# dhruvsreenivas/amp_extensions

Measured on AMD Instinct MI355X. Metric: learned-dynamics env steps/sec (humanoid3d, 40k-sample rollout), higher is better.
Workload: dtype fp32 (f16x3-emulated: 2 scaled fp16 limbs, 3 MFMA products per f32 MAC, fp32-level error)

## Files before the change

### amp_extensions_amd/_native.py

```python
from __future__ import annotations

import ctypes as C
import os
import re

from . import _build

_HEADER = os.path.join(_build.INCLUDE, "amx_hip.h")
ABI_VERSION = 2

c_int, c_ll, c_dbl, c_flt, c_u64, c_u32, vp = C.c_int, C.c_longlong, C.c_double, C.c_float, C.c_uint64, C.c_uint32, C.c_void_p
ip = C.POINTER(C.c_int)


class ResetNoise(C.Structure):
    _fields_ = [("noise_bef_rot", C.c_int), ("noise_min", C.c_double), ("noise_max", C.c_double),
                ("radian", C.c_double), ("rot_vel_w_pose", C.c_int), ("vel_noise", C.c_int),
                ("interp", C.c_double), ("knee_rot", C.c_int)]

    @classmethod
    def from_reset_args(cls, ra: dict) -> "ResetNoise | None":
        if float(ra["radian"]) == 0 and float(ra["noise_min"]) == 0 and float(ra["noise_max"]) == 0:
            return None
        return cls(int(bool(ra["noise_bef_rot"])), float(ra["noise_min"]), float(ra["noise_max"]),
                   float(ra["radian"]), int(bool(ra["rot_vel_w_pose"])), int(bool(ra["vel_noise"])),
                   float(ra["interp"]), int(bool(ra["knee_rot"])))


AMX_NOISE_ROT_SLOTS = 48
RFF_PART_ROWS = 32

SIGNATURES = {
    "amx_create": (vp, [c_int, c_int, c_int, c_int, c_int, c_int, c_int]),
    "amx_create_ex": (vp, [c_int, c_int, c_int, c_int, c_int, c_int, c_int, c_int]),
    "amx_destroy": (c_int, [vp]),
    "amx_last_error": (C.c_char_p, []),
    "amx_abi_version": (c_int, []),
    "amx_layout": (c_int, [vp, ip, ip, ip, ip]),
    "amx_set_normalizers": (c_int, [vp, vp, vp, vp, vp, vp, vp]),
    "amx_set_termination": (c_int, [vp, c_int, vp, vp, vp, vp, c_int, c_int, c_int, c_int, c_int,
                                    c_int, c_int, c_dbl, c_int, c_dbl]),
    "amx_assemble_input": (c_int, [vp, vp, vp, c_int, vp, c_ll, c_int, c_int, vp]),
    "amx_assemble_input_rexp": (c_int, [vp, vp, vp, c_int, vp, c_ll, c_int, c_int, vp, c_ll, c_ll, c_int, vp]),
    "amx_gemm_bias_act": (c_int, [vp, c_int, c_int, c_int, c_int, vp, c_int, c_ll, vp, c_int, c_ll,
                                  vp, c_ll, vp, c_int, c_ll, c_int, c_int, vp]),
    "amx_gemm_bias_act_t64": (c_int, [vp, c_int, c_int, c_int, c_int, vp, c_int, c_ll, vp, c_int, c_ll,
                                      vp, c_ll, vp, c_int, c_ll, c_int, c_int, vp]),
    "amx_gemm_out_unnorm": (c_int, [vp, c_int, c_int, c_int, c_int, vp, c_int, c_ll, vp, c_int, c_ll,
                                    vp, c_ll, vp, c_int, c_ll, vp]),
    "amx_split_bf16x3": (c_int, [vp, c_int, c_int, c_int, vp, c_int, c_ll, vp, c_ll, vp]),
    "amx_gemm_bias_act_x6": (c_int, [vp, c_int, c_int, c_int, c_int, vp, c_int, c_ll, vp, c_ll,
                                     vp, c_ll, vp, c_int, c_ll, c_int, c_int, vp]),
    "amx_gemm_out_unnorm_x6": (c_int, [vp, c_int, c_int, c_int, c_int, vp, c_int, c_ll, vp, c_ll,
                                       vp, c_ll, vp, c_int, c_ll, vp]),
    "amx_rff_features_x6": (c_int, [vp, c_int, c_int, c_int, c_int, vp, c_int, vp, vp, c_flt, vp, c_int,
                                    vp, vp, vp]),
    "amx_split_f16x2": (c_int, [vp, c_int, c_int, c_int, vp, c_int, c_ll, vp, c_ll, vp, c_ll, vp]),
    "amx_row_exponents": (c_int, [vp, c_int, c_int, c_int, vp, c_int, c_ll, vp, c_ll, c_int, vp]),
    "amx_gemm_bias_act_h3": (c_int, [vp, c_int, c_int, c_int, c_int, vp, c_int, c_ll, vp, c_ll, vp, c_ll,
                                     vp, c_ll, vp, c_int, c_ll, c_int, c_int, vp, c_ll, c_int, vp, c_int, vp]),
    "amx_gemm_out_unnorm_h3": (c_int, [vp, c_int, c_int, c_int, c_int, vp, c_int, c_ll, vp, c_ll, vp, c_ll,
                                       vp, c_ll, vp, c_int, c_ll, vp, c_ll, c_int, c_int, vp]),
    "amx_gemm_bias_act_h3_win": (c_int, [vp, c_int, c_int, c_int, c_int, vp, c_int, c_ll, vp, c_ll, vp, c_ll,
                                         vp, c_ll, vp, c_int, c_ll, c_int, c_int, vp, c_ll, c_int, vp, c_int, vp]),
    "amx_gemm_out_unnorm_h3_win": (c_int, [vp, c_int, c_int, c_int, c_int, vp, c_int, c_ll, vp, c_ll, vp, c_ll,
                                           vp, c_ll, vp, c_int, c_ll, vp, c_ll, c_int, vp]),
    "amx_set_motion": (c_int, [vp, vp, c_ll]),
    "amx_motion_duration": (c_dbl, [vp]),
    "amx_motion_states": (c_int, [vp, vp, c_int, c_int, vp, c_ll, vp]),
    "amx_motion_states_noise": (c_int, [vp, vp, c_int, c_int, vp, vp, c_ll, c_u64, vp, c_ll, vp]),
    "amx_reset_lanes_motion_noise": (c_int, [vp, vp, vp, c_u64, c_dbl, c_int, vp, vp, c_ll, vp, vp, vp, vp, vp, vp,
                                             c_int, vp]),
    "amx_reset_lanes_motion": (c_int, [vp, vp, vp, c_u64, c_dbl, c_int, vp, vp, vp, vp, vp, vp, c_int, vp]),
    "amx_amp_obs_size": (c_int, [vp]),
    "amx_state_amp_obs": (c_int, [vp, vp, vp, c_ll, c_int, c_int, vp, c_ll, vp]),
    "amx_motion_amp_obs": (c_int, [vp, vp, c_dbl, c_int, c_int, vp, c_ll, vp]),
    "amx_state_amp_rows": (c_int, [vp, vp, vp, c_ll, c_int, c_int, vp, c_ll, vp]),
    "amx_tw_dim": (c_int, [vp]),
    "amx_state_tw_rows": (c_int, [vp, vp, c_ll, c_int, c_int, vp, c_ll, vp]),
    "amx_motion_tw_rows": (c_int, [vp, vp, vp, c_int, c_int, c_dbl, vp, c_ll, vp]),
    "amx_dtw_work": (c_ll, [c_int, c_int]),
    "amx_dtw_align": (c_int, [vp, vp, vp, c_ll, c_int, c_int, c_int, vp, vp, c_int, c_int, vp, vp, vp, vp, vp, vp, vp]),
    "amx_npg_param_count": (c_ll, [c_int, c_int]),
    "amx_npg_pass": (c_int, [vp, c_int, c_int, vp, c_int, c_ll, vp, c_int, c_ll, vp, vp, vp, c_int, vp, vp]),
    "amx_npg_reduce": (c_int, [vp, vp, c_int, c_int, vp, vp]),
    "amx_npg_pass_gated": (c_int, [vp, c_int, c_int, vp, c_int, c_ll, vp, c_int, c_ll, vp, vp, vp, c_int, vp, vp, vp]),
    "amx_npg_reduce_gated": (c_int, [vp, vp, c_int, c_int, vp, vp, vp]),
    "amx_npg_curvature": (c_int, [vp, vp, c_int, c_int, vp, vp]),
    "amx_npg_cg_tail_work": (c_ll, [c_int]),
    "amx_npg_cg_tail": (c_int, [vp, vp, c_int, c_int, c_int, vp, c_dbl, c_dbl, vp, vp, vp, vp, vp, vp, vp, vp, vp]),
    "amx_npg_cg_reduce": (c_int, [vp, vp, c_int, c_int, c_int, vp, c_dbl, vp, vp, vp, vp, vp]),
    "amx_npg_cg_xrp": (c_int, [vp, c_int, c_dbl, vp, vp, vp, vp, vp, vp, vp, vp, vp]),
    "amx_npg_pass_cg": (c_int, [vp, c_int, vp, c_int, c_ll, vp, c_int, vp, vp, c_dbl, vp, vp, vp, vp, vp, vp, vp, vp,
                                vp, vp]),
    "amx_npg_pass_idx": (c_int, [vp, c_int, c_int, vp, vp, c_int, c_ll, vp, vp, c_int, vp, vp, vp, vp, vp]),
    "amx_npg_pass_cg_idx": (c_int, [vp, c_int, c_int, vp, vp, c_int, c_ll, vp, c_int, vp, vp, c_dbl, vp, vp, vp, vp,
                                    vp, vp, vp, vp, vp, vp, vp]),
    "amx_npg_ll_blocks": (c_int, [vp, c_int]),
    "amx_npg_ll": (c_int, [vp, c_int, vp, c_ll, vp, c_ll, vp, vp, vp, vp, vp]),
    "amx_npg_apply_step": (c_int, [vp, c_int, c_int, vp, vp, vp, c_int, c_dbl, c_dbl, c_flt, vp, vp, vp]),
    "amx_npg_pass_ex": (c_int, [vp, c_int, c_int, vp, c_int, c_ll, vp, c_int, c_ll, vp, vp, vp, c_int, vp, vp, vp, vp]),
    "amx_npg_pass_dp": (c_int, [vp, c_int, c_int, vp, c_int, c_ll, vp, c_int, c_ll, vp, vp, vp, c_int, vp, vp, vp, c_ll,
                                vp]),
    "amx_npg_pass_cg_dp": (c_int, [vp, c_int, vp, c_int, c_ll, vp, c_int, vp, vp, c_dbl, vp, vp, vp, vp, vp, vp, vp,
                                   vp, vp, c_ll, vp]),
    "amx_npg_cg_init": (c_int, [vp, c_int, vp, vp, vp, vp, vp, vp, vp]),
    "amx_npg_cg_init_ls": (c_int, [vp, c_int, c_int, vp, vp, vp, vp, vp, vp, vp, vp, vp]),
    "amx_npg_cg_step": (c_int, [vp, c_int, c_int, vp, vp, c_dbl, c_dbl, vp, vp, vp, vp, vp, vp]),
    "amx_step": (c_int, [vp, vp, c_int, c_ll, vp, vp, vp, vp, vp, vp, vp, c_int, vp, c_int, vp]),
    "amx_step_rexp": (c_int, [vp, vp, c_int, c_ll, vp, vp, vp, vp, vp, vp, vp, c_int, vp, vp, c_int, vp]),
    "amx_step_reset": (c_int, [vp, vp, c_int, c_ll, vp, vp, vp, vp, vp, vp, vp, c_int, vp, vp, vp, c_int, vp,
                               c_u64, vp, vp, vp, vp, vp, c_ll, vp, c_int, vp]),
    "amx_step_reset_act": (c_int, [vp, vp, c_int, c_ll, vp, vp, vp, vp, vp, vp, vp, c_int, vp, vp, vp, c_int, vp,
                                   c_u64, vp, vp, vp, vp, vp, vp, c_int, c_int, vp, c_u64, c_u64, vp, c_int, vp, vp,
                                   vp, c_ll, c_int, vp, c_ll, c_ll, c_int, c_int, vp]),
    "amx_set_step_act_occupancy": (c_int, [vp, c_int]),
    "amx_rff_features_h3": (c_int, [vp, c_int, c_int, c_int, c_int, vp, c_int, vp, vp, vp, vp, c_flt, vp, c_int,
                                    vp, vp, vp]),
    "amx_mlp_features_h3": (c_int, [vp, c_int, c_int, c_int, c_int, vp, c_int, vp, vp, vp, vp, c_flt, vp, c_int,
                                    vp, vp, vp]),
    "amx_disagreement": (c_int, [vp, vp, c_int, c_ll, vp, c_int, vp]),
    "amx_reset_lanes": (c_int, [vp, vp, vp, c_int, vp, c_u64, vp, vp, vp, vp, vp, vp, c_int, vp]),
    "amx_policy_act": (c_int, [vp, vp, c_int, vp, c_int, c_int, vp, vp, c_u64, c_u64, c_int, vp, vp, vp, c_ll,
                               c_int, vp, c_ll, c_ll, c_int, vp]),
    "amx_policy_act_dev": (c_int, [vp, vp, c_int, vp, c_int, c_int, vp, vp, c_u64, vp, c_u64, c_int, vp, vp, vp,
                                   c_ll, c_int, vp, c_ll, c_ll, c_int, vp]),
    "amx_counter_add": (c_int, [vp, vp, c_ll, vp]),
    "amx_set_gemm_timer": (c_int, [vp, vp]),
    "amx_split_workspace_floats": (c_ll, [vp, c_int, c_int, ip]),
    "amx_set_split_workspace": (c_int, [vp, vp, c_ll, vp, c_int]),
    "amx_policy_blob_floats": (c_ll, [vp, c_int, c_int]),
    "amx_policy_pack": (c_int, [vp, vp, vp, c_int, vp, vp, c_int, vp, vp, vp, vp]),
    "amx_rff_features": (c_int, [vp, c_int, c_int, c_int, c_int, vp, c_int, vp, c_int, vp, c_flt, vp, c_int,
                                 vp, vp, vp]),
    "amx_sum_partials": (c_int, [vp, vp, c_int, c_int, vp, vp]),
    "amx_mmd_fit": (c_int, [vp, vp, c_dbl, vp, c_int, vp, vp, vp]),
    "amx_mmd_reward": (c_int, [vp, vp, c_int, vp, c_int, vp, c_flt, c_dbl, c_flt, c_flt, vp, vp, vp, c_int, vp]),
    "amx_mmd_reward_raw": (c_int, [vp, vp, c_int, vp, c_int, vp, c_dbl, vp, vp, vp, c_int, vp]),
    "amx_expert_cost": (c_int, [vp, vp, c_int, vp, c_int, c_int, c_flt, c_flt, vp, vp, c_dbl, vp]),
    "amx_feature_message": (c_int, [vp, vp, c_int, c_int, c_dbl, vp, vp]),
    "amx_mmd_relabel": (c_int, [vp, vp, c_dbl, vp, c_int, vp, vp, vp, c_int, vp, c_flt, c_dbl, c_int, c_flt, c_flt,
                                vp, vp, vp, c_int, vp, c_int, c_int, vp, vp, vp, vp]),
    "amx_amp_reward": (c_int, [vp, vp, c_int, c_int, vp, c_flt, vp, c_dbl, vp, vp, c_int, vp]),
    "amx_disc_reward": (c_int, [vp, c_int, vp, c_int, c_int, vp, c_flt, vp, c_dbl, vp, vp, c_int, vp]),
    "amx_cost_rows": (c_int, [vp, vp, c_ll, c_int, vp, c_ll, c_int, vp, c_ll, c_int, c_int, vp, c_int, vp]),
    "amx_value_features": (c_int, [vp, c_int, c_int, vp, vp, vp, c_ll, vp, vp, c_int, vp, c_int, vp]),
    "amx_value_head": (c_int, [vp, c_int, vp, c_int, c_int, vp, vp, vp, vp]),
    "amx_gae": (c_int, [vp, c_int, c_int, vp, vp, c_ll, vp, vp, vp, c_ll, vp, c_dbl, c_dbl, vp, vp, vp]),
    "amx_adv_whiten": (c_int, [vp, c_int, c_int, vp, vp, c_ll, vp, c_dbl, vp, vp, vp]),
    "amx_adv_whiten_parts": (c_int, [vp, c_int, c_int, vp, vp, c_ll, vp, c_int, c_int, vp, vp]),
    "amx_adv_whiten_apply": (c_int, [vp, c_int, c_int, vp, vp, c_ll, vp, vp, c_int, c_dbl, vp, vp, vp]),
    "amx_vfit_work": (c_ll, [c_int, c_int, c_int]),
    "amx_vfit_param_count": (c_ll, [c_int, c_int, c_int]),
    "amx_vfit_epoch": (c_int, [vp, c_int, vp, c_int, vp, vp, c_int, c_int, c_int, vp, vp, vp, vp, vp, vp, vp, vp, vp,
                               c_dbl, c_dbl, c_dbl, c_dbl, c_dbl, vp, vp, vp]),
    "amx_efit_param_count": (c_ll, [vp]),
    "amx_efit_work_floats": (c_ll, [vp, c_int]),
    "amx_efit_step": (c_int, [vp, c_int, c_int, c_int, vp, c_ll, c_int, vp, vp, vp, vp, vp, vp, vp, vp, vp, c_int,
                              c_dbl, c_dbl, c_dbl, vp, c_ll, vp, vp]),
    "amx_gemm_nn_f32": (c_int, [vp, c_int, c_int, c_int, vp, c_int, vp, c_int, vp, c_int, vp, c_int, c_int, vp]),
    "amx_gemm_tn_f32": (c_int, [vp, c_int, c_int, c_int, vp, c_int, vp, c_int, vp, c_int, vp, c_int, vp, c_int, vp]),
    "amx_dfit_param_count": (c_ll, [c_int, c_int, c_int]),
    "amx_dfit_work_floats": (c_ll, [c_int, c_int, c_int, c_int]),
    "amx_dfit_step": (c_int, [vp, c_int, c_int, c_dbl, c_dbl, c_dbl, c_dbl, c_dbl, c_int, c_int, c_int, c_int, c_int,
                              c_int, vp, vp, vp, c_ll, c_int, vp, c_ll, c_int, vp, vp, vp, vp, vp, vp, vp, vp, vp, vp,
                              vp, vp]),
    "amx_bcfit_work": (c_ll, [c_int, c_int]),
    "amx_bcfit_steps": (c_int, [vp, c_int, vp, c_ll, vp, c_ll, vp, c_int, vp, vp, vp, vp, c_dbl, c_dbl, c_dbl, c_dbl,
                                c_dbl, c_int, vp, vp]),
    "amx_bcfit_eval": (c_int, [vp, c_int, vp, c_ll, vp, c_ll, vp, c_int, vp, vp, vp]),
    "amx_ppo_steps": (c_int, [vp, c_int, vp, c_ll, vp, c_ll, vp, vp, vp, c_int, vp, c_int, vp, vp, vp, vp, c_dbl, c_dbl,
                              c_dbl, c_dbl, c_dbl, vp, vp, vp]),
    "amx_ppo_old_ll": (c_int, [vp, c_int, vp, c_ll, vp, c_ll, vp, vp, vp]),
    "amx_philox":(c_int, [vp, c_u64, c_u32, c_u32, c_u32, vp, c_int, vp]),
    "amx_mt_seed": (c_int, [vp, c_int, vp, vp, c_int]),
    "amx_mt_policy_noise": (c_int, [vp, c_int, vp, c_int, c_int, c_int, vp, c_ll, c_ll]),
}
AMX_MT_STATE_BYTES = 2512

AMX_ROW_TILE = 128
AMX_K_TILE = 32
AMX_SHAPE_SPHERE, AMX_SHAPE_CAPSULE, AMX_SHAPE_BOX = 0, 1, 2
AMX_ACT_NONE, AMX_ACT_RELU = 0, 1
AMX_CONNECT_DENSE, AMX_CONNECT_PLAIN = 0, 1
AMX_IN_F64, AMX_IN_F32 = 0, 1
AMX_DISC_LEAST_SQUARES, AMX_DISC_LOG_LIKELIHOOD = 0, 1
AMX_EFIT_ADAM, AMX_EFIT_SGD = 0, 1
AMX_DFIT_SGD, AMX_DFIT_ADAM = 0, 1
AMX_BC_MSE, AMX_BC_MLE = 0, 1
AMX_DTW_COST_SQUARED, AMX_DTW_COST_POINTS = 0, 1
AMX_PPO_OLD_SNAPSHOT, AMX_PPO_OLD_TRACKS_MEAN = 0, 1


class AmxNativeError(RuntimeError):
    pass


def header_symbols(path: str = _HEADER) -> list[str]:
    txt = open(path).read()
    txt = re.sub(r"/\*.*?\*/", "", txt, flags=re.S)
    return sorted(set(re.findall(r"\b(amx_[a-z0-9_]+)\s*\(", txt)))


_LIB = None


def load(path: str | None = None, build_if_missing: bool = False):
    global _LIB
    if _LIB is not None and path is None:
        return _LIB
    path = path or _build.LIB_PATH
    if not os.path.exists(path):
        if build_if_missing:
            _build.build()
        else:
            raise AmxNativeError(
                f"{path} is missing: build it with `python -m amp_extensions_amd._build` "
                "(there is no CPU fallback for the rollout hot path)")
    try:
        lib = C.CDLL(path, mode=C.RTLD_GLOBAL)
    except OSError as e:
        raise AmxNativeError(f"cannot load {path}: {e}") from e
    for name, (res, args) in SIGNATURES.items():
        fn = getattr(lib, name)
        fn.restype = res
        fn.argtypes = args
    if lib.amx_abi_version() != ABI_VERSION:
        raise AmxNativeError("libamx_hip ABI version mismatch")
    if path == _build.LIB_PATH:
        _LIB = lib
    return lib


def check(rc: int, what: str = "") -> None:
    if rc != 0:
        msg = _LIB.amx_last_error().decode() if _LIB is not None else "?"
        raise AmxNativeError(f"{what or 'amx call'} failed ({rc}): {msg}")


def ptr(t) -> int | None:
    if t is None:
        return None
    return t.data_ptr()


def stream_handle(device=None) -> int:
    import torch
    return torch.cuda.current_stream(device).cuda_stream
```

### amp_extensions_amd/csrc/amx_step.hip

```cpp
#include "amx_common.h"

#include <utility>
#include <stdlib.h>

namespace {

template <int CTRL, int RM>
__device__ __forceinline__ double dpp_f64(double v) {
  const int lo = __builtin_amdgcn_update_dpp(0, __double2loint(v), CTRL, RM, 0xf, false);
  const int hi = __builtin_amdgcn_update_dpp(0, __double2hiint(v), CTRL, RM, 0xf, false);
  return __hiloint2double(hi, lo);
}

__device__ inline double wave_sum(double v) {
  v += dpp_f64<0xb1, 0xf>(v);
  v += dpp_f64<0x4e, 0xf>(v);
  v += dpp_f64<0x141, 0xf>(v);
  v += dpp_f64<0x140, 0xf>(v);
  v += dpp_f64<0x142, 0xa>(v);
  v += dpp_f64<0x143, 0xc>(v);
  const int lo = __builtin_amdgcn_readlane(__double2loint(v), 63);
  const int hi = __builtin_amdgcn_readlane(__double2hiint(v), 63);
  return __hiloint2double(hi, lo);
}

template <typename T>
__global__ __launch_bounds__(256) void k_assemble(const T* __restrict__ ob, const T* __restrict__ act,
                                                  const float* __restrict__ norm, float* __restrict__ buf,
                                                  long long stride_m, int ldk, int S, int A, int M, int k0_pad,
                                                  int B, int* __restrict__ row_exp, long long stride_rexp,
                                                  long long slot_stride, int n_slots) {
  const int b = (blockIdx.x * blockDim.x + threadIdx.x) >> 6;
  const int lane = threadIdx.x & 63;
  if (b >= B) return;
  const float* mu_s = norm;
  const float* sd_s = norm + S;
  const float* mu_a = norm + 2 * S;
  const float* sd_a = norm + 2 * S + A;
  uint32_t mx = 0;
  const int copies = stride_m == 0 ? 1 : M;
  for (int j = lane; j < k0_pad; j += 64) {
    float x = 0.f;
    if (j < S) {
      const float s = (float)ob[(long long)b * S + j];
      x = (s - mu_s[j]) / sd_s[j];
    } else if (j < S + A) {
      const int k = j - S;
      const float v = (float)act[(long long)b * A + k];
      x = (v - mu_a[k]) / sd_a[k];
    }
    for (int m = 0; m < copies; ++m) buf[m * stride_m + (long long)b * ldk + j] = x;
    const uint32_t bits = __float_as_uint(x) & 0x7fffffffu;
    mx = mx > bits ? mx : bits;
  }
  if (row_exp == nullptr) return;
#pragma unroll
  for (int off = 32; off > 0; off >>= 1) {
    const uint32_t o = (uint32_t)__shfl_xor((int)mx, off);
    mx = mx > o ? mx : o;
  }
  if (lane < n_slots) {
    int e = (int)(mx >> 23) - 126;
    e = e < -100 ? -100 : (e > 100 ? 100 : e);
    const int v = lane == 0 ? e : -100;
    if (slot_stride < B) {
      const int Bq = (int)slot_stride, g = b / Bq;
      row_exp[g * stride_rexp + lane * slot_stride + (b - g * Bq)] = v;
    } else {
      for (int m = 0; m < M; ++m) row_exp[m * stride_rexp + lane * slot_stride + b] = v;
    }
  }
}

template <int MM>
__device__ inline float lane_disagreement(const float* __restrict__ preds, long long strideP, int ldp, int b,
                                          int S, int lane) {
  constexpr int NP = MM * (MM - 1) / 2;
  double acc[NP > 0 ? NP : 1];
#pragma unroll
  for (int p = 0; p < (NP > 0 ? NP : 1); ++p) acc[p] = 0.0;
  for (int j = lane; j < S; j += 64) {
    float v[MM];
#pragma unroll
    for (int m = 0; m < MM; ++m) v[m] = preds[m * strideP + (long long)b * ldp + j];
    int p = 0;
#pragma unroll
    for (int i = 0; i < MM; ++i)
#pragma unroll
      for (int k = i + 1; k < MM; ++k) {
        const float d = v[i] - v[k];
        acc[p++] += (double)d * (double)d;
      }
  }
  double best = 0.0;
#pragma unroll
  for (int p = 0; p < NP; ++p) {
    const double n = wave_sum(acc[p]);
    best = (p == 0 || n > best) ? n : best;
  }
  return (float)sqrt(best);
}

__device__ inline float lane_disagreement_any(const float* __restrict__ preds, long long strideP, int ldp, int b,
                                              int S, int M, int lane) {
  double best = 0.0;
  bool first = true;
  for (int i = 0; i < M; ++i)
    for (int k = i + 1; k < M; ++k) {
      double acc = 0.0;
      for (int j = lane; j < S; j += 64) {
        const float d = preds[i * strideP + (long long)b * ldp + j] - preds[k * strideP + (long long)b * ldp + j];
        acc += (double)d * (double)d;
      }
      const double n = wave_sum(acc);
      best = (first || n > best) ? n : best;
      first = false;
    }
  return (float)sqrt(best);
}

__device__ inline float disagreement_dispatch(int M, const float* preds, long long strideP, int ldp, int b, int S,
                                              int lane) {
  if (M == 4) return lane_disagreement<4>(preds, strideP, ldp, b, S, lane);
  return M >= 2 ? lane_disagreement_any(preds, strideP, ldp, b, S, M, lane) : 0.f;
}

__global__ __launch_bounds__(256) void k_disagreement(const float* __restrict__ preds, long long strideP, int ldp,
                                                      float* __restrict__ disc, int S, int M, int B) {
  const int b = (blockIdx.x * blockDim.x + threadIdx.x) >> 6;
  const int lane = threadIdx.x & 63;
  if (b >= B) return;
  const float d = disagreement_dispatch(M, preds, strideP, ldp, b, S, lane);
  if (lane == 0) disc[b] = d;
}

struct StepArgs {
  const float* preds; long long strideP; int ldp;
  const int32_t* model_idx; int32_t* model_idx_out;
  const double* ob; double* ob_next;
  int32_t* num_steps; uint8_t* done; float* disc;
  float* cost_in; int ldc;
  int* cost_rexp;
  uint8_t* nonfinite;
  int S, M, B;
  amx_termination term;
  double* ob_out; const double* table; int R; const int32_t* rows; uint32_t k0, k1;
  int32_t* reset_count; int32_t* row_out;
  int32_t* steps0_out;
  uint64_t* counter; long long counter_delta;
  double* ob_rec;
};

template <int NIT, bool MM4>
__device__ __forceinline__ void step_lane(const StepArgs& a, int b, int lane, float* srow) {
  const amx_termination& T = a.term;
  const int S = a.S;
  const int k = a.model_idx[b];
  const int ns0 = a.num_steps[b];
  const int rc0 = a.ob_out ? a.reset_count[b] : 0;
  const int row0 = (a.ob_out && a.rows) ? a.rows[b] : 0;
  const double* ob = a.ob + (long long)b * S;
  double* on = a.ob_next + (long long)b * S;

  double o[NIT], x[NIT];
  float p[NIT];
  float pm[MM4 ? 4 : 1][NIT];
  if constexpr (MM4) {
    const float* pb = a.preds + (long long)b * a.ldp;
#pragma unroll
    for (int it = 0; it < NIT; ++it) {
      const int j = lane + 64 * it;
      o[it] = j < S ? ob[j] : 0.0;
#pragma unroll
      for (int m = 0; m < 4; ++m) pm[m][it] = j < S ? pb[m * a.strideP + j] : 0.f;
    }
#pragma unroll
    for (int it = 0; it < NIT; ++it)
      p[it] = k == 0 ? pm[0][it] : k == 1 ? pm[1][it] : k == 2 ? pm[2][it] : pm[3][it];
  } else {
    const float* pk = a.preds + (long long)k * a.strideP + (long long)b * a.ldp;
#pragma unroll
    for (int it = 0; it < NIT; ++it) {
      const int j = lane + 64 * it;
      o[it] = j < S ? ob[j] : 0.0;
      p[it] = j < S ? pk[j] : 0.f;
    }
  }
  const bool vscale = T.vel_check && T.record_vel_as_pos;
  bool vel_bad = false, bad = false;
  uint32_t cmax = 0;
#pragma unroll
  for (int it = 0; it < NIT; ++it) {
    const int j = lane + 64 * it;
    double v = o[it] + (double)p[it];
    if (vscale && j >= T.vel_offset) v = v / T.sampling_rate;
    x[it] = v;
    if (j < S) {
      on[j] = v;
      if (a.ob_rec) a.ob_rec[(long long)b * S + j] = o[it];
      if (T.vel_check && j >= T.vel_offset) vel_bad |= fabs(v) > T.vel_thresh;
      bad |= !isfinite(v);
      if (a.cost_in) {
        const float c0 = (float)o[it], c1 = (float)v;
        a.cost_in[(long long)b * a.ldc + j] = c0;
        a.cost_in[(long long)b * a.ldc + S + j] = c1;
        const uint32_t u0 = __float_as_uint(c0) & 0x7fffffffu, u1 = __float_as_uint(c1) & 0x7fffffffu;
        cmax = cmax > u0 ? cmax : u0;
        cmax = cmax > u1 ? cmax : u1;
      }
    }
  }
  if (a.cost_in) {
    for (int j = 2 * S + lane; j < a.ldc; j += 64) a.cost_in[(long long)b * a.ldc + j] = 0.f;
    if (a.cost_rexp) {
#pragma unroll
      for (int off = 32; off > 0; off >>= 1) {
        const uint32_t oo = (uint32_t)__shfl_xor((int)cmax, off);
        cmax = cmax > oo ? cmax : oo;
      }
      if (lane == 0) {
        int e = (int)(cmax >> 23) - 126;
        a.cost_rexp[b] = e < -100 ? -100 : (e > 100 ? 100 : e);
      }
    }
  }

  auto fetch = [&](int j) -> double {
    const int src = j & 63, itj = j >> 6;
    double r = 0.0;
#pragma unroll
    for (int it = 0; it < NIT; ++it) {
      const double v = __shfl(x[it], src);
      r = (itj == it) ? v : r;
    }
    return r;
  };
  const int bi = lane < T.n ? lane : 0;
  const double root_y = fetch(0);
  const double rel_y = fetch(T.y_index[bi]);
  const double ny = fetch(T.shape[bi] == AMX_SHAPE_CAPSULE ? T.ny_index[bi] : 0);
  bool hit = false;
  if (lane < T.n && (T.shape[bi] == AMX_SHAPE_SPHERE || T.shape[bi] == AMX_SHAPE_CAPSULE)) {
    const double y = T.list_index_world[bi] ? rel_y : root_y + rel_y;
    if (T.shape[bi] == AMX_SHAPE_SPHERE) {
      hit = y <= T.thresh[bi];
    } else {
      const double top = T.half_h[bi] * ny;
      const double bot = T.neg_half_h[bi] * ny;
      const double ytop = y + top;
      const double ybot = y + bot;
      hit = (ytop <= T.thresh[bi]) || (ybot <= T.thresh[bi]);
    }
  }
  const bool collided = __ballot(hit) != 0ull;
  const bool vexp = __ballot(vel_bad) != 0ull;
  const bool nf = __ballot(bad) != 0ull;

  float d = 0.f;
  if constexpr (MM4) {
    if (a.disc) {
      double acc[6] = {0.0, 0.0, 0.0, 0.0, 0.0, 0.0};
#pragma unroll
      for (int it = 0; it < NIT; ++it) {
        if (lane + 64 * it < S) {
          int q = 0;
#pragma unroll
          for (int i = 0; i < 4; ++i)
#pragma unroll
            for (int kk = i + 1; kk < 4; ++kk) {
              const float df = pm[i][it] - pm[kk][it];
              acc[q++] += (double)df * (double)df;
            }
        }
      }
      double mx = 0.0;
#pragma unroll
      for (int q = 0; q < 6; ++q) {
        const double n = wave_sum(acc[q]);
        mx = (q == 0 || n > mx) ? n : mx;
      }
      d = (float)sqrt(mx);
    }
  } else {
    if (a.disc) d = disagreement_dispatch(a.M, a.preds, a.strideP, a.ldp, b, S, lane);
  }

  const int ns = ns0 + 1;
  const bool horizon_done = ns >= T.horizon;
  const bool dn = horizon_done || collided || vexp;
  bool reset = false;
  if (a.ob_out) {
    double* oo = a.ob_out + (long long)b * S;
    if (!dn) {
#pragma unroll
      for (int it = 0; it < NIT; ++it) {
        const int j = lane + 64 * it;
        if (j < S) {
          oo[j] = x[it];
          if (srow) srow[j] = (float)x[it];
        }
      }
      if (lane == 0 && a.row_out) a.row_out[b] = -1;
    } else {
      reset = true;
      const int rc = rc0 + 1;
      int row;
      if (a.rows) {
        row = row0;
      } else {
        const amx::u32x4 r = amx::philox4x32_10({(uint32_t)b, (uint32_t)rc, 0u, amx::kTagReset}, a.k0, a.k1);
        row = (int)((((uint64_t)r.y << 32) | r.x) % (uint64_t)a.R);
      }
      const double* src = a.table + (long long)row * S;
      for (int j = lane; j < S; j += 64) {
        const double v = src[j];
        oo[j] = v;
        if (srow) srow[j] = (float)v;
      }
      if (lane == 0) {
        a.reset_count[b] = rc;
        a.model_idx_out[b] = rc % a.M;
        if (a.row_out) a.row_out[b] = row;
      }
    }
  }

  if (a.counter && b == 0 && lane == 0) a.counter[0] += (uint64_t)a.counter_delta;
  if (lane == 0) {
    if (a.steps0_out) a.steps0_out[b] = ns - 1;
    a.num_steps[b] = reset ? 0 : ns;
    a.done[b] = dn ? 1 : 0;
    if (a.disc) a.disc[b] = d;
    if (a.nonfinite) a.nonfinite[b] = nf ? 1 : 0;
  }
}

template <int NIT, bool MM4>
__global__ __launch_bounds__(256) void k_step(StepArgs a) {
  const int b = (blockIdx.x * blockDim.x + threadIdx.x) >> 6;
  const int lane = threadIdx.x & 63;
  if (b >= a.B) return;
  step_lane<NIT, MM4>(a, b, lane, nullptr);
}

__global__ __launch_bounds__(256) void k_reset(const uint8_t* __restrict__ mask, const double* __restrict__ table,
                                               int R, const int32_t* __restrict__ rows, uint32_t k0, uint32_t k1,
                                               const double* ob_src, double* ob_out, int32_t* num_steps,
                                               int32_t* model_idx, int32_t* reset_count, int32_t* row_out, int S,
                                               int M, int B) {
  const int b = (blockIdx.x * blockDim.x + threadIdx.x) >> 6;
  const int lane = threadIdx.x & 63;
  if (b >= B) return;
  const bool do_reset = (mask == nullptr) || mask[b] != 0;
  if (!do_reset) {
    if (ob_src != ob_out)
      for (int j = lane; j < S; j += 64) ob_out[(long long)b * S + j] = ob_src[(long long)b * S + j];
    if (lane == 0 && row_out) row_out[b] = -1;
    return;
  }
  const int rc = reset_count[b] + 1;
  int row;
  if (rows) {
    row = rows[b];
  } else {
    const amx::u32x4 r = amx::philox4x32_10({(uint32_t)b, (uint32_t)rc, 0u, amx::kTagReset}, k0, k1);
    const uint64_t x = ((uint64_t)r.y << 32) | r.x;
    row = (int)(x % (uint64_t)R);
  }
  const double* src = table + (long long)row * S;
  for (int j = lane; j < S; j += 64) ob_out[(long long)b * S + j] = src[j];
  if (lane == 0) {
    reset_count[b] = rc;
    model_idx[b] = rc % M;
    num_steps[b] = 0;
    if (row_out) row_out[b] = row;
  }
}

constexpr int POL_LANES = 16;
constexpr int POL_MAXH = 256;
constexpr int POL_X0_COLS = 320;

__host__ __device__ inline int pol_stride(int k) {
  const int r = (k + 3) & ~3;
  return (r % 8 == 0) ? r + 4 : r;
}

__host__ __device__ inline int pol_blob_floats(int S, int H1, int H2, int A) {
  const int s1 = pol_stride(S), s2 = pol_stride(H1), s3 = pol_stride(H2);
  return (H1 * s1 + H2 * s2 + A * s3 + H1 + H2 + A + 3) & ~3;
}

__host__ __device__ inline int pol_part_floats(int H1, int H2, int A) {
  int h = H1 > H2 ? H1 : H2;
  h = h > A ? h : A;
  const int w = 16 * ((h + 15) / 16);
  return POL_LANES * (w > 64 ? w : 64);
}

__host__ inline size_t pol_lds_bytes(int S, int H1, int H2, int A) {
  const int s1 = pol_stride(S), s2 = pol_stride(H1), s3 = pol_stride(H2);
  const size_t fl = (size_t)pol_blob_floats(S, H1, H2, A) + POL_LANES * (s1 + s2 + s3 + 2 * A) +
                    pol_part_floats(H1, H2, A);
  return fl * sizeof(float);
}

struct PolicyArgs {
  const double* ob; const float* blob; int H1; int H2; const double* nscale; const double* noise;
  uint32_t k0, k1, ctr_lo, ctr_hi; int eval_mode;
  const uint64_t* ctr_dev;
  double* act; float* mean_out;
  float* x0; long long stride_m; int ldk; int k0_pad; int M; const float* norm;
  int* row_exp; long long stride_rexp; long long slot_stride; int n_slots;
  int S, A, B;
};

typedef float pf4 __attribute__((ext_vector_type(4)));

constexpr int POL_STAGE_W = 12;
constexpr int POL_STAGE_O = 16;

__device__ inline void pol_zero_pads(float* __restrict__ dst, int ds, int cols, int rows) {
  const int w = ds - cols;
  for (int i = threadIdx.x; i < rows * w; i += 256) dst[(i / w) * ds + cols + i % w] = 0.f;
}

__device__ inline void pol_stage_all(float* __restrict__ img, const float* __restrict__ blob, int n4,
                                     float* __restrict__ so, int s1, const double* __restrict__ ob, int n_ob,
                                     int S) {
  const int t = threadIdx.x;
  for (int it = 0;; ++it) {
    const int w0 = t + it * 256 * POL_STAGE_W, o0 = t + it * 256 * POL_STAGE_O;
    if (w0 >= n4 && o0 >= n_ob) break;
    pf4 wv[POL_STAGE_W];
    double ov[POL_STAGE_O];
#pragma unroll
    for (int u = 0; u < POL_STAGE_W; ++u) {
      const int i = w0 + u * 256;
      if (i < n4) wv[u] = reinterpret_cast<const pf4*>(blob)[i];
    }
#pragma unroll
    for (int u = 0; u < POL_STAGE_O; ++u) {
      const int i = o0 + u * 256;
      if (i < n_ob) ov[u] = ob[i];
    }
#pragma unroll
    for (int u = 0; u < POL_STAGE_W; ++u) {
      const int i = w0 + u * 256;
      if (i < n4) reinterpret_cast<pf4*>(img)[i] = wv[u];
    }
#pragma unroll
    for (int u = 0; u < POL_STAGE_O; ++u) {
      const int i = o0 + u * 256;
      if (i < n_ob) {
        const int r = i / S, c = i - r * S;
        so[r * s1 + c] = (float)ov[u];
      }
    }
  }
}

__device__ inline int pol_ksplit(int nblk, int nc) {
  const int jjt = (nc + 3) >> 2;
  return nblk >= 4 ? 1 : (4 / nblk < jjt ? 4 / nblk : jjt);
}

__device__ inline void pol_mfma_layer(const float* __restrict__ x, int ldx, int nc, const float* __restrict__ w,
                                      int ldw, int N, float* __restrict__ part) {
  const int lane = threadIdx.x & 63, wave = threadIdx.x >> 6;
  const int i = lane & 15, kq = lane >> 4;
  const int nblk = (N + 15) >> 4, jjt = (nc + 3) >> 2, ksplit = pol_ksplit(nblk, nc);
  const int ldp = 16 * nblk;
  for (int item = wave; item < nblk * ksplit; item += 4) {
    const int nb = item % nblk, kh = item / nblk;
    const int jj0 = kh * jjt / ksplit, jj1 = (kh + 1) * jjt / ksplit;
    const int u = 16 * nb + i;
    const float* xr = x + i * ldx;
    const float* wr = w + (u < N ? u : 0) * ldw;
    pf4 acc = {0.f, 0.f, 0.f, 0.f};
    for (int jj = jj0; jj < jj1; ++jj) {
      const int c = kq + 4 * jj;
      const bool ok = c < nc;
      const pf4 a = ok ? *reinterpret_cast<const pf4*>(xr + 4 * c) : pf4{0.f, 0.f, 0.f, 0.f};
      const pf4 b = (ok && u < N) ? *reinterpret_cast<const pf4*>(wr + 4 * c) : pf4{0.f, 0.f, 0.f, 0.f};
      acc = __builtin_amdgcn_mfma_f32_16x16x4f32(a.x, b.x, acc, 0, 0, 0);
      acc = __builtin_amdgcn_mfma_f32_16x16x4f32(a.y, b.y, acc, 0, 0, 0);
      acc = __builtin_amdgcn_mfma_f32_16x16x4f32(a.z, b.z, acc, 0, 0, 0);
      acc = __builtin_amdgcn_mfma_f32_16x16x4f32(a.w, b.w, acc, 0, 0, 0);
    }
    float* pp = part + kh * 16 * ldp + 16 * nb + i;
#pragma unroll
    for (int r = 0; r < 4; ++r) pp[(4 * kq + r) * ldp] = acc[r];
  }
}

__device__ inline void pol_combine(const float* __restrict__ part, int N, int nc, const float* __restrict__ bias,
                                   bool tanh_act, float* __restrict__ out, int ldo) {
  const int nblk = (N + 15) >> 4, ksplit = pol_ksplit(nblk, nc), ldp = 16 * nblk;
  for (int e = threadIdx.x; e < POL_LANES * N; e += 256) {
    const int l = e / N, u = e - l * N;
    float z = part[l * ldp + u];
    for (int kh = 1; kh < ksplit; ++kh) z += part[(kh * 16 + l) * ldp + u];
    z = z + bias[u];
    out[l * ldo + u] = tanh_act ? tanhf(z) : z;
  }
}

__device__ __forceinline__ void policy_core(const PolicyArgs& p, float* psm, int b0, int img_floats) {
  const int S = p.S, A = p.A, H1 = p.H1, H2 = p.H2;
  const int s1 = pol_stride(S), s2 = pol_stride(H1), s3 = pol_stride(H2);
  float* w1 = psm;
  float* w2 = w1 + H1 * s1;
  float* w3 = w2 + H2 * s2;
  float* bb1 = w3 + A * s3;
  float* bb2 = bb1 + H1;
  float* bb3 = bb2 + H2;
  float* so = psm + img_floats;
  float* h1 = so + POL_LANES * s1;
  float* h2 = h1 + POL_LANES * s2;
  float* mo = h2 + POL_LANES * s3;
  float* xa_s = mo + POL_LANES * A;
  float* part = xa_s + POL_LANES * A;
  const int t = threadIdx.x;
  const bool on = t < 256;
  const int nc1 = (S + 3) >> 2, nc2 = (H1 + 3) >> 2, nc3 = (H2 + 3) >> 2;
  const int npairs = (A + 1) >> 1;
  constexpr int POL_PRE = 2;
  double pre_n[POL_PRE][2], pre_s[POL_PRE][2];
#pragma unroll
  for (int q = 0; q < POL_PRE; ++q) {
    const int e = t + 256 * q;
    const int l = e / npairs, pr = e - l * npairs, b = b0 + l;
#pragma unroll
    for (int h = 0; h < 2; ++h) {
      const int u = 2 * pr + h;
      const bool ok = on && e < POL_LANES * npairs && b < p.B && u < A;
      pre_n[q][h] = (ok && p.noise && !p.eval_mode) ? p.noise[(long long)b * A + u] : 0.0;
      pre_s[q][h] = (ok && !p.eval_mode) ? p.nscale[u] : 0.0;
    }
  }
  if (on) pol_mfma_layer(so, s1, nc1, w1, s1, H1, part);
  __syncthreads();
  if (on) pol_combine(part, H1, nc1, bb1, true, h1, s2);
  __syncthreads();
  if (on) pol_mfma_layer(h1, s2, nc2, w2, s2, H2, part);
  __syncthreads();
  if (on) pol_combine(part, H2, nc2, bb2, true, h2, s3);
  __syncthreads();
  if (on) pol_mfma_layer(h2, s3, nc3, w3, s3, A, part);
  __syncthreads();
  if (on) pol_combine(part, A, nc3, bb3, false, mo, A);
  __syncthreads();
  uint32_t ctr_lo = p.ctr_lo, ctr_hi = p.ctr_hi;
  if (p.ctr_dev) {
    const uint64_t cv = *p.ctr_dev + ((uint64_t)p.ctr_hi << 32 | p.ctr_lo);
    ctr_lo = (uint32_t)cv;
    ctr_hi = (uint32_t)(cv >> 32);
  }
  auto act_item = [&](int e, const double* pn, const double* ps) {
    const int l = e / npairs, pr = e - l * npairs;
    const int b = b0 + l;
    if (b >= p.B) return;
    double n[2] = {0.0, 0.0};
    if (!p.eval_mode && !p.noise) {
      const amx::u32x4 r = amx::philox4x32_10(
          {(uint32_t)b, ctr_lo, ((uint32_t)pr << 8) | (ctr_hi & 0xffu), amx::kTagPolicy}, p.k0, p.k1);
      const double u1 = 1.0 - amx::u53(r.x, r.y);
      const double u2 = amx::u53(r.z, r.w);
      const double rad = sqrt(-2.0 * log(u1));
      const double ang = 6.283185307179586 * u2;
      n[0] = rad * cos(ang);
      n[1] = rad * sin(ang);
    }
#pragma unroll
    for (int h = 0; h < 2; ++h) {
      const int u = 2 * pr + h;
      if (u >= A) break;
      const float m = mo[l * A + u];
      if (p.mean_out) p.mean_out[(long long)b * A + u] = m;
      double a_out;
      if (p.eval_mode) {
        a_out = (double)m;
      } else {
        const double nz = p.noise ? (pn ? pn[h] : p.noise[(long long)b * A + u]) : n[h];
        a_out = (double)m + (ps ? ps[h] : p.nscale[u]) * nz;
      }
      p.act[(long long)b * A + u] = a_out;
      if (p.x0) xa_s[l * A + u] = (float)a_out;
    }
  };
  if (on) {
#pragma unroll
    for (int q = 0; q < POL_PRE; ++q)
      if (t + 256 * q < POL_LANES * npairs) act_item(t + 256 * q, pre_n[q], pre_s[q]);
    for (int e = t + 256 * POL_PRE; e < POL_LANES * npairs; e += 256) act_item(e, nullptr, nullptr);
  }
  if (!p.x0) return;
  __syncthreads();
  if (!on) return;
  const float* mu_s = p.norm;
  const float* sd_s = p.norm + S;
  const float* mu_a = p.norm + 2 * S;
  const float* sd_a = p.norm + 2 * S + A;
  const int k0 = p.k0_pad;
  const int copies = p.stride_m == 0 ? 1 : p.M;
  const int ll = t >> 4, c0 = t & 15;
  const int bb = b0 + ll;
  const bool row_ok = bb < p.B;
  constexpr int QT = POL_X0_COLS / 16;
  float mu[QT], sd[QT];
#pragma unroll
  for (int q = 0; q < QT; ++q) {
    const int j = c0 + 16 * q;
    mu[q] = 0.f;
    sd[q] = 1.f;
    if (j < S) {
      mu[q] = mu_s[j];
      sd[q] = sd_s[j];
    } else if (j < S + A) {
      mu[q] = mu_a[j - S];
      sd[q] = sd_a[j - S];
    }
  }
  uint32_t mx = 0;
  if (row_ok) {
#pragma unroll
    for (int q = 0; q < QT; ++q) {
      const int j = c0 + 16 * q;
      if (j >= k0) break;
      float x = 0.f;
      if (j < S) {
        x = (so[ll * s1 + j] - mu[q]) / sd[q];
      } else if (j < S + A) {
        x = (xa_s[ll * A + j - S] - mu[q]) / sd[q];
      }
      for (int mm = 0; mm < copies; ++mm) p.x0[mm * p.stride_m + (long long)bb * p.ldk + j] = x;
      const uint32_t bits = __float_as_uint(x) & 0x7fffffffu;
      mx = mx > bits ? mx : bits;
    }
  }
  if (p.row_exp == nullptr) return;
#pragma unroll
  for (int off = 8; off > 0; off >>= 1) {
    const uint32_t o = (uint32_t)__shfl_xor((int)mx, off);
    mx = mx > o ? mx : o;
  }
  if (!row_ok) return;
  int e = (int)(mx >> 23) - 126;
  e = e < -100 ? -100 : (e > 100 ? 100 : e);
  for (int sl = c0; sl < p.n_slots; sl += 16) {
    const int v = sl == 0 ? e : -100;
    if (p.slot_stride < p.B) {
      const int Bq = (int)p.slot_stride, g = bb / Bq;
      p.row_exp[g * p.stride_rexp + sl * p.slot_stride + (bb - g * Bq)] = v;
    } else {
      for (int mm = 0; mm < p.M; ++mm) p.row_exp[mm * p.stride_rexp + sl * p.slot_stride + bb] = v;
    }
  }
}


__global__ __launch_bounds__(256) void k_policy(PolicyArgs p) {
  extern __shared__ __attribute__((aligned(16))) float psm[];
  const int S = p.S, s1 = pol_stride(S), s2 = pol_stride(p.H1), s3 = pol_stride(p.H2);
  const int nblob = pol_blob_floats(S, p.H1, p.H2, p.A);
  float* so = psm + nblob;
  float* h1 = so + POL_LANES * s1;
  const int t = threadIdx.x;
  const int b0 = blockIdx.x * POL_LANES;
  const int nl = (p.B - b0) < POL_LANES ? (p.B - b0) : POL_LANES;
  pol_zero_pads(so, s1, S, nl);
  for (int i = t + nl * s1; i < POL_LANES * s1; i += 256) so[i] = 0.f;
  pol_stage_all(psm, p.blob, nblob >> 2, so, s1, p.ob + (long long)b0 * S, nl * S, S);
  for (int i = t; i < POL_LANES * (s2 + s3); i += 256) h1[i] = 0.f;
  __syncthreads();
  policy_core(p, psm, b0, nblob);
}

__host__ __device__ inline int pol_image_lds_floats(int S, int H1, int H2, int A) {
  return (pol_blob_floats(S, H1, H2, A) + 255) & ~255;
}

template <int NIT, bool MM4, bool W8>
__global__ __launch_bounds__(1024) __attribute__((amdgpu_waves_per_eu(W8 ? 8 : 1))) void k_step_act(StepArgs a,
                                                                                                    PolicyArgs p) {
  extern __shared__ __attribute__((aligned(16))) float psm[];
  const int S = p.S, s1 = pol_stride(S), s2 = pol_stride(p.H1), s3 = pol_stride(p.H2);
  const int nimg = pol_image_lds_floats(S, p.H1, p.H2, p.A);
  float* so = psm + nimg;
  float* h1 = so + POL_LANES * s1;
  const int t = threadIdx.x, lane = t & 63, wave = t >> 6;
  const int b0 = blockIdx.x * POL_LANES, b = b0 + wave;
  for (int q = wave; q < (nimg >> 8); q += POL_LANES)
    __builtin_amdgcn_global_load_lds((const __attribute__((address_space(1))) void*)(p.blob + q * 256 + 4 * lane),
                                     (__attribute__((address_space(3))) void*)(psm + q * 256), 16, 0, 0);
  float* srow = so + wave * s1;
  if (b < a.B) {
    step_lane<NIT, MM4>(a, b, lane, srow);
    for (int j = S + lane; j < s1; j += 64) srow[j] = 0.f;
  } else {
    for (int j = lane; j < s1; j += 64) srow[j] = 0.f;
  }
  for (int i = t; i < POL_LANES * (s2 + s3); i += 1024) h1[i] = 0.f;
  __syncthreads();
  policy_core(p, psm, b0, nimg);
}

__global__ void k_policy_pack(const float* __restrict__ W1, const float* __restrict__ b1, int H1,
                              const float* __restrict__ W2, const float* __restrict__ b2, int H2,
                              const float* __restrict__ W3, const float* __restrict__ b3, int S, int A,
                              float* __restrict__ blob) {
  const int s1 = pol_stride(S), s2 = pol_stride(H1), s3 = pol_stride(H2);
  const int n = pol_blob_floats(S, H1, H2, A);
  const int i = blockIdx.x * blockDim.x + threadIdx.x;
  if (i >= n) return;
  int j = i;
  float v = 0.f;
  if (j < H1 * s1) {
    const int r = j / s1, c = j % s1;
    v = c < S ? W1[(long long)r * S + c] : 0.f;
  } else if ((j -= H1 * s1) < H2 * s2) {
    const int r = j / s2, c = j % s2;
    v = c < H1 ? W2[r * H1 + c] : 0.f;
  } else if ((j -= H2 * s2) < A * s3) {
    const int r = j / s3, c = j % s3;
    v = c < H2 ? W3[r * H2 + c] : 0.f;
  } else if ((j -= A * s3) < H1) {
    v = b1[j];
  } else if ((j -= H1) < H2) {
    v = b2[j];
  } else if ((j -= H2) < A) {
    v = b3[j];
  }
  blob[i] = v;
}

__global__ void k_philox(uint32_t k0, uint32_t k1, uint32_t c1, uint32_t c2, uint32_t c3, uint32_t* out, int n) {
  const int i = blockIdx.x * blockDim.x + threadIdx.x;
  if (i >= n) return;
  const amx::u32x4 r = amx::philox4x32_10({(uint32_t)i, c1, c2, c3}, k0, k1);
  out[4 * i + 0] = r.x;
  out[4 * i + 1] = r.y;
  out[4 * i + 2] = r.z;
  out[4 * i + 3] = r.w;
}

inline dim3 lanes_grid(int B) { return dim3((unsigned)((B + 3) / 4)); }

}

static bool blocked_rexp_ok(const amx_ctx* ctx, int B, long long stride_m, long long stride_rexp, long long slot_stride,
                            int n_slots) {
  return ctx && stride_m == 0 && slot_stride > 0 && B % slot_stride == 0 && B / slot_stride <= ctx->M &&
         stride_rexp >= (long long)n_slots * slot_stride;
}

static int assemble(const char* fn, amx_ctx* ctx, const void* ob, const void* act, int in_dtype, float* act_buf,
                    long long stride_m, int ldk, int B, int* row_exp, long long stride_rexp, long long slot_stride,
                    int n_slots, void* stream) {
  AMX_CHECK_ARG(ctx && ctx->have_norm, "%s: context has no normalizers", fn);
  AMX_CHECK_ARG(ob && act && act_buf, "%s: null pointer", fn);
  AMX_CHECK_ARG(B >= 0, "%s: B=%d", fn, B);
  AMX_CHECK_ARG(ldk >= ctx->k0_pad, "%s: ldk=%d < k0_pad=%d", fn, ldk, ctx->k0_pad);
  AMX_CHECK_ARG(ctx->M == 1 || stride_m == 0 || stride_m >= (long long)ldk * B, "%s: stride_m too small", fn);
  if (B == 0) return AMX_OK;
  hipStream_t s = (hipStream_t)stream;
  if (in_dtype == AMX_IN_F64) {
    hipLaunchKernelGGL(k_assemble<double>, lanes_grid(B), dim3(256), 0, s, (const double*)ob, (const double*)act,
                       ctx->d_norm, act_buf, stride_m, ldk, ctx->S, ctx->A, ctx->M, ctx->k0_pad, B, row_exp,
                       stride_rexp, slot_stride, n_slots);
  } else if (in_dtype == AMX_IN_F32) {
    hipLaunchKernelGGL(k_assemble<float>, lanes_grid(B), dim3(256), 0, s, (const float*)ob, (const float*)act,
                       ctx->d_norm, act_buf, stride_m, ldk, ctx->S, ctx->A, ctx->M, ctx->k0_pad, B, row_exp,
                       stride_rexp, slot_stride, n_slots);
  } else {
    AMX_CHECK_ARG(false, "%s: in_dtype=%d", fn, in_dtype);
  }
  AMX_CHECK_LAUNCH();
  return AMX_OK;
}

extern "C" int amx_assemble_input(amx_ctx* ctx, const void* ob, const void* act, int in_dtype, float* act_buf,
                                  long long stride_m, int ldk, int B, void* stream) {
  return assemble("amx_assemble_input", ctx, ob, act, in_dtype, act_buf, stride_m, ldk, B, nullptr, 0, 0, 0,
                  stream);
}

extern "C" int amx_assemble_input_rexp(amx_ctx* ctx, const void* ob, const void* act, int in_dtype, float* act_buf,
                                       long long stride_m, int ldk, int B, int* row_exp, long long strideRexp,
                                       long long slot_stride, int n_slots, void* stream) {
  AMX_CHECK_ARG(row_exp && n_slots >= 1 && n_slots <= 64 &&
                    (slot_stride >= B ? (ctx == nullptr || ctx->M == 1 || strideRexp >= (long long)n_slots * slot_stride)
                                      : blocked_rexp_ok(ctx, B, stride_m, strideRexp, slot_stride, n_slots)),
                "amx_assemble_input_rexp: row_exp=%p n_slots=%d slot_stride=%lld strideRexp=%lld B=%d", (void*)row_exp,
                n_slots, slot_stride, strideRexp, B);
  return assemble("amx_assemble_input_rexp", ctx, ob, act, in_dtype, act_buf, stride_m, ldk, B, row_exp, strideRexp,
                  slot_stride, n_slots, stream);
}

static int make_policy_args(const char* fn, amx_ctx* ctx, const double* ob, int B, const float* blob, int H1, int H2,
                            const double* noise_scale, const double* noise, uint64_t seed, uint64_t counter,
                            const uint64_t* counter_dev, int eval_mode, double* act, float* mean, float* x0_buf,
                            long long stride_m, int ldk, int* row_exp, long long stride_rexp, long long slot_stride,
                            int n_slots, PolicyArgs& p) {
  AMX_CHECK_ARG(ctx && blob && act, "%s: null pointer", fn);
  AMX_CHECK_ARG(amx::aligned16(blob), "%s: blob must be 16-byte aligned", fn);
  AMX_CHECK_ARG(eval_mode || noise_scale, "%s: noise_scale required unless eval_mode", fn);
  AMX_CHECK_ARG(H1 > 0 && H1 <= POL_MAXH && H2 > 0 && H2 <= POL_MAXH && ctx->A <= POL_MAXH && ctx->S <= POL_MAXH,
                "%s: S=%d H1=%d H2=%d A=%d (max %d)", fn, ctx->S, H1, H2, ctx->A, POL_MAXH);
  AMX_CHECK_ARG(B >= 0, "%s: B=%d", fn, B);
  AMX_CHECK_ARG(!x0_buf || ctx->k0_pad <= POL_X0_COLS, "%s: fused assembly needs k0_pad <= %d (%d)", fn,
                POL_X0_COLS, ctx->k0_pad);
  AMX_CHECK_ARG(!x0_buf || (ctx->have_norm && ldk >= ctx->k0_pad &&
                            (ctx->M == 1 || stride_m == 0 || stride_m >= (long long)ldk * B)),
                "%s: fused assembly needs normalizers and ldk >= k0_pad, stride_m >= ldk*B", fn);
  AMX_CHECK_ARG(!row_exp || (x0_buf && n_slots >= 1 && n_slots <= 64 &&
                             (slot_stride >= B ? (ctx->M == 1 || stride_rexp >= (long long)n_slots * slot_stride)
                                               : blocked_rexp_ok(ctx, B, stride_m, stride_rexp, slot_stride, n_slots))),
                "%s: row_exp needs x0_buf, 1 <= n_slots <= 64, slot_stride >= B (or the member-blocked layout), "
                "stride_rexp", fn);
  const size_t lds = pol_lds_bytes(ctx->S, H1, H2, ctx->A);
  AMX_CHECK_ARG(lds <= 160 * 1024, "%s: S/H too large for LDS staging (%zu B)", fn, lds);
  p.ob = ob; p.blob = blob; p.H1 = H1; p.H2 = H2;
  p.nscale = noise_scale; p.noise = noise;
  p.k0 = (uint32_t)seed; p.k1 = (uint32_t)(seed >> 32); p.ctr_lo = (uint32_t)counter;
  p.ctr_hi = (uint32_t)(counter >> 32); p.eval_mode = eval_mode; p.ctr_dev = counter_dev;
  p.act = act; p.mean_out = mean;
  p.x0 = x0_buf; p.stride_m = stride_m; p.ldk = ldk; p.k0_pad = ctx->k0_pad; p.M = ctx->M; p.norm = ctx->d_norm;
  p.row_exp = row_exp; p.stride_rexp = stride_rexp; p.slot_stride = slot_stride; p.n_slots = n_slots;
  p.S = ctx->S; p.A = ctx->A; p.B = B;
  return AMX_OK;
}

static int policy_act(amx_ctx* ctx, const double* ob, int B, const float* blob, int H1, int H2,
                      const double* noise_scale, const double* noise, uint64_t seed, uint64_t counter,
                      const uint64_t* counter_dev, int eval_mode, double* act, float* mean, float* x0_buf,
                      long long stride_m, int ldk, int* row_exp, long long stride_rexp, long long slot_stride,
                      int n_slots, void* stream) {
  AMX_CHECK_ARG(ob, "amx_policy_act: null ob");
  PolicyArgs p;
  const int rc = make_policy_args("amx_policy_act", ctx, ob, B, blob, H1, H2, noise_scale, noise, seed, counter,
                                  counter_dev, eval_mode, act, mean, x0_buf, stride_m, ldk, row_exp, stride_rexp,
                                  slot_stride, n_slots, p);
  if (rc) return rc;
  if (B == 0) return AMX_OK;
  hipLaunchKernelGGL(k_policy, dim3((B + POL_LANES - 1) / POL_LANES), dim3(256), pol_lds_bytes(ctx->S, H1, H2, ctx->A),
                     (hipStream_t)stream, p);
  AMX_CHECK_LAUNCH();
  return AMX_OK;
}

struct ResetArgs {
  const double* table; int R; const int32_t* rows; uint64_t seed; double* ob_out; int32_t* model_idx;
  int32_t* reset_count; int32_t* row_out; int32_t* steps0_out;
  uint64_t* counter; long long counter_delta; double* ob_rec;
};

static int step_impl(amx_ctx* ctx, const float* preds, int ldp, long long strideP, const int32_t* model_idx,
                     const double* ob, double* ob_next, int32_t* num_steps, uint8_t* done, float* disc,
                     float* cost_in, int ldc, int* cost_rexp, uint8_t* nonfinite, int B, void* stream,
                     const ResetArgs* rs = nullptr, const PolicyArgs* pa = nullptr) {
  AMX_CHECK_ARG(ctx && ctx->have_term, "amx_step: context has no termination config");
  AMX_CHECK_ARG(preds && model_idx && ob && ob_next && num_steps && done, "amx_step: null pointer");
  AMX_CHECK_ARG(ldp >= ctx->S && B >= 0, "amx_step: ldp=%d B=%d", ldp, B);
  AMX_CHECK_ARG(!disc || ctx->M >= 2, "amx_step: disagreement needs >= 2 models");
  AMX_CHECK_ARG(!cost_in || ldc >= 2 * ctx->S, "amx_step: ldc=%d < 2S", ldc);
  AMX_CHECK_ARG(ob != ob_next, "amx_step: ob and ob_next must not alias");
  if (B == 0) return AMX_OK;
  StepArgs a;
  a.preds = preds; a.strideP = strideP; a.ldp = ldp;
  a.model_idx = model_idx; a.ob = ob; a.ob_next = ob_next;
  a.num_steps = num_steps; a.done = done; a.disc = disc;
  a.cost_in = cost_in; a.ldc = ldc; a.cost_rexp = cost_rexp; a.nonfinite = nonfinite;
  a.S = ctx->S; a.M = ctx->M; a.B = B; a.term = ctx->term;
  a.model_idx_out = nullptr; a.ob_out = nullptr; a.table = nullptr; a.R = 0; a.rows = nullptr; a.k0 = a.k1 = 0;
  a.reset_count = nullptr; a.row_out = nullptr; a.steps0_out = nullptr; a.counter = nullptr; a.counter_delta = 0;
  a.ob_rec = nullptr;
  if (rs) {
    AMX_CHECK_ARG(rs->table && rs->ob_out && rs->model_idx && rs->reset_count && rs->R > 0,
                  "amx_step_reset: null reset pointer or R=%d", rs->R);
    AMX_CHECK_ARG(rs->ob_out != ob_next && (const int32_t*)rs->model_idx == model_idx,
                  "amx_step_reset: ob_out must differ from ob_next and model_idx be the step's");
    AMX_CHECK_ARG(rs->ob_rec == nullptr || (rs->ob_rec != ob && rs->ob_rec != ob_next && rs->ob_rec != rs->ob_out),
                  "amx_step_reset: ob_rec must be a fourth buffer");
    a.model_idx_out = rs->model_idx; a.ob_out = rs->ob_out; a.table = rs->table; a.R = rs->R; a.rows = rs->rows;
    a.k0 = (uint32_t)rs->seed; a.k1 = (uint32_t)(rs->seed >> 32);
    a.reset_count = rs->reset_count; a.row_out = rs->row_out; a.steps0_out = rs->steps0_out;
    a.counter = rs->counter; a.counter_delta = rs->counter_delta; a.ob_rec = rs->ob_rec;
  }
  const int nit = (ctx->S + 63) / 64;
  if (pa) {
    AMX_CHECK_ARG(rs && !rs->counter && !pa->noise && pa->B == B && nit <= 4,
                  "amx_step_reset_act: needs the table reset, no counter advance, no injected noise, S <= 256");
    const size_t lds = pol_lds_bytes(ctx->S, pa->H1, pa->H2, ctx->A) +
                       (size_t)(pol_image_lds_floats(ctx->S, pa->H1, pa->H2, ctx->A) -
                                pol_blob_floats(ctx->S, pa->H1, pa->H2, ctx->A)) * sizeof(float);
    AMX_CHECK_ARG(lds <= 160 * 1024, "amx_step_reset_act: S/H too large for LDS staging (%zu B)", lds);
    const dim3 grid((B + POL_LANES - 1) / POL_LANES);
    switch (nit) {
#define AMX_STEP_ACT_CASE(N)                                                                                       \
  case N:                                                                                                          \
    if (ctx->M == 4 && ctx->step_act_w8) hipLaunchKernelGGL((k_step_act<N, true, true>), grid, dim3(1024), lds,     \
                                                           (hipStream_t)stream, a, *pa);                          \
    else if (ctx->M == 4) hipLaunchKernelGGL((k_step_act<N, true, false>), grid, dim3(1024), lds, (hipStream_t)stream, \
                                             a, *pa);                                                              \
    else hipLaunchKernelGGL((k_step_act<N, false, false>), grid, dim3(1024), lds, (hipStream_t)stream, a, *pa);   \
    break;
      AMX_STEP_ACT_CASE(1) AMX_STEP_ACT_CASE(2) AMX_STEP_ACT_CASE(3) AMX_STEP_ACT_CASE(4)
#undef AMX_STEP_ACT_CASE
    }
    AMX_CHECK_LAUNCH();
    return AMX_OK;
  }
  switch (nit) {
#define AMX_STEP_CASE(N)                                                                                 \
  case N:                                                                                                \
    if (ctx->M == 4) hipLaunchKernelGGL((k_step<N, true>), lanes_grid(B), dim3(256), 0, (hipStream_t)stream, a); \
    else hipLaunchKernelGGL((k_step<N, false>), lanes_grid(B), dim3(256), 0, (hipStream_t)stream, a);     \
    break;
    AMX_STEP_CASE(1) AMX_STEP_CASE(2) AMX_STEP_CASE(3) AMX_STEP_CASE(4)
    AMX_STEP_CASE(5) AMX_STEP_CASE(6) AMX_STEP_CASE(7) AMX_STEP_CASE(8)
#undef AMX_STEP_CASE
    default: AMX_CHECK_ARG(false, "amx_step: S=%d exceeds 512", ctx->S);
  }
  AMX_CHECK_LAUNCH();
  return AMX_OK;
}

extern "C" int amx_step(amx_ctx* ctx, const float* preds, int ldp, long long strideP, const int32_t* model_idx,
                        const double* ob, double* ob_next, int32_t* num_steps, uint8_t* done, float* disc,
                        float* cost_in, int ldc, uint8_t* nonfinite, int B, void* stream) {
  return step_impl(ctx, preds, ldp, strideP, model_idx, ob, ob_next, num_steps, done, disc, cost_in, ldc, nullptr,
                   nonfinite, B, stream);
}

extern "C" int amx_step_rexp(amx_ctx* ctx, const float* preds, int ldp, long long strideP, const int32_t* model_idx,
                             const double* ob, double* ob_next, int32_t* num_steps, uint8_t* done, float* disc,
                             float* cost_in, int ldc, int* cost_rexp, uint8_t* nonfinite, int B, void* stream) {
  AMX_CHECK_ARG(cost_in && cost_rexp, "amx_step_rexp: cost_in and cost_rexp are required");
  return step_impl(ctx, preds, ldp, strideP, model_idx, ob, ob_next, num_steps, done, disc, cost_in, ldc, cost_rexp,
                   nonfinite, B, stream);
}

extern "C" int amx_step_reset(amx_ctx* ctx, const float* preds, int ldp, long long strideP, int32_t* model_idx,
                              const double* ob, double* ob_next, int32_t* num_steps, uint8_t* done, float* disc,
                              float* cost_in, int ldc, int* cost_rexp, uint8_t* nonfinite, const double* table,
                              int R, const int32_t* rows, uint64_t seed, double* ob_out, int32_t* reset_count,
                              int32_t* row_out, int32_t* steps0_out, uint64_t* counter, long long counter_delta,
                              double* ob_rec, int B, void* stream) {
  AMX_CHECK_ARG(!cost_rexp || cost_in, "amx_step_reset: cost_rexp needs cost_in");
  const ResetArgs rs = {table, R, rows, seed, ob_out, model_idx, reset_count, row_out, steps0_out, counter,
                        counter_delta, ob_rec};
  return step_impl(ctx, preds, ldp, strideP, model_idx, ob, ob_next, num_steps, done, disc, cost_in, ldc, cost_rexp,
                   nonfinite, B, stream, &rs);
}

extern "C" int amx_step_reset_act(amx_ctx* ctx, const float* preds, int ldp, long long strideP, int32_t* model_idx,
                                  const double* ob, double* ob_next, int32_t* num_steps, uint8_t* done, float* disc,
                                  float* cost_in, int ldc, int* cost_rexp, uint8_t* nonfinite, const double* table,
                                  int R, const int32_t* rows, uint64_t seed, double* ob_out, int32_t* reset_count,
                                  int32_t* row_out, int32_t* steps0_out, double* ob_rec, const float* blob, int H1,
                                  int H2, const double* noise_scale, uint64_t policy_seed, uint64_t counter,
                                  const uint64_t* counter_dev, int eval_mode, double* act, float* mean,
                                  float* x0_buf, long long stride_m, int ldk, int* row_exp, long long stride_rexp,
                                  long long slot_stride, int n_slots, int B, void* stream) {
  AMX_CHECK_ARG(!cost_rexp || cost_in, "amx_step_reset_act: cost_rexp needs cost_in");
  PolicyArgs p;
  int rc = make_policy_args("amx_step_reset_act", ctx, nullptr, B, blob, H1, H2, noise_scale, nullptr, policy_seed,
                            counter, counter_dev, eval_mode, act, mean, x0_buf, stride_m, ldk, row_exp, stride_rexp,
                            slot_stride, n_slots, p);
  if (rc) return rc;
  const ResetArgs rs = {table, R, rows, seed, ob_out, model_idx, reset_count, row_out, steps0_out, nullptr, 0,
                        ob_rec};
  return step_impl(ctx, preds, ldp, strideP, model_idx, ob, ob_next, num_steps, done, disc, cost_in, ldc, cost_rexp,
                   nonfinite, B, stream, &rs, &p);
}

extern "C" int amx_disagreement(amx_ctx* ctx, const float* preds, int ldp, long long strideP, float* disc, int B,
                                void* stream) {
  AMX_CHECK_ARG(ctx && preds && disc, "amx_disagreement: null pointer");
  AMX_CHECK_ARG(ctx->M >= 2, "amx_disagreement: needs >= 2 models (M=%d)", ctx->M);
  AMX_CHECK_ARG(ldp >= ctx->S && B >= 0, "amx_disagreement: ldp=%d B=%d", ldp, B);
  if (B == 0) return AMX_OK;
  hipLaunchKernelGGL(k_disagreement, lanes_grid(B), dim3(256), 0, (hipStream_t)stream, preds, strideP, ldp, disc,
                     ctx->S, ctx->M, B);
  AMX_CHECK_LAUNCH();
  return AMX_OK;
}

extern "C" int amx_reset_lanes(amx_ctx* ctx, const uint8_t* mask, const double* table, int R, const int32_t* rows,
                               uint64_t seed, const double* ob_src, double* ob_out, int32_t* num_steps,
                               int32_t* model_idx, int32_t* reset_count, int32_t* row_out, int B, void* stream) {
  AMX_CHECK_ARG(ctx && table && ob_out && num_steps && model_idx && reset_count, "amx_reset_lanes: null pointer");
  AMX_CHECK_ARG(R > 0 && B >= 0, "amx_reset_lanes: R=%d B=%d", R, B);
  AMX_CHECK_ARG(mask == nullptr || ob_src != nullptr, "amx_reset_lanes: masked reset needs ob_src");
  if (B == 0) return AMX_OK;
  hipLaunchKernelGGL(k_reset, lanes_grid(B), dim3(256), 0, (hipStream_t)stream, mask, table, R, rows,
                     (uint32_t)seed, (uint32_t)(seed >> 32), ob_src, ob_out, num_steps, model_idx, reset_count,
                     row_out, ctx->S, ctx->M, B);
  AMX_CHECK_LAUNCH();
  return AMX_OK;
}

extern "C" long long amx_policy_blob_floats(const amx_ctx* ctx, int H1, int H2) {
  if (!ctx || H1 <= 0 || H2 <= 0) return -1;
  return pol_image_lds_floats(ctx->S, H1, H2, ctx->A);
}

extern "C" int amx_policy_pack(amx_ctx* ctx, const float* W1, const float* b1, int H1, const float* W2,
                               const float* b2, int H2, const float* W3, const float* b3, float* blob,
                               void* stream) {
  AMX_CHECK_ARG(ctx && W1 && b1 && W2 && b2 && W3 && b3 && blob, "amx_policy_pack: null pointer");
  AMX_CHECK_ARG(H1 > 0 && H1 <= POL_MAXH && H2 > 0 && H2 <= POL_MAXH && ctx->A <= POL_MAXH,
                "amx_policy_pack: H1=%d H2=%d A=%d (max %d)", H1, H2, ctx->A, POL_MAXH);
  AMX_CHECK_ARG(amx::aligned16(blob), "amx_policy_pack: blob must be 16-byte aligned");
  const int n = pol_blob_floats(ctx->S, H1, H2, ctx->A);
  hipLaunchKernelGGL(k_policy_pack, dim3((n + 255) / 256), dim3(256), 0, (hipStream_t)stream, W1, b1, H1, W2, b2,
                     H2, W3, b3, ctx->S, ctx->A, blob);
  AMX_CHECK_LAUNCH();
  return AMX_OK;
}

extern "C" int amx_policy_act(amx_ctx* ctx, const double* ob, int B, const float* blob, int H1, int H2,
                              const double* noise_scale, const double* noise, uint64_t seed, uint64_t counter,
                              int eval_mode, double* act, float* mean, float* x0_buf, long long stride_m, int ldk,
                              int* row_exp, long long stride_rexp, long long slot_stride, int n_slots,
                              void* stream) {
  return policy_act(ctx, ob, B, blob, H1, H2, noise_scale, noise, seed, counter, nullptr, eval_mode, act, mean,
                    x0_buf, stride_m, ldk, row_exp, stride_rexp, slot_stride, n_slots, stream);
}

extern "C" int amx_policy_act_dev(amx_ctx* ctx, const double* ob, int B, const float* blob, int H1, int H2,
                                  const double* noise_scale, const double* noise, uint64_t seed,
                                  const uint64_t* counter, uint64_t counter_offset, int eval_mode, double* act,
                                  float* mean, float* x0_buf, long long stride_m, int ldk, int* row_exp,
                                  long long stride_rexp, long long slot_stride, int n_slots, void* stream) {
  AMX_CHECK_ARG(counter, "amx_policy_act_dev: null counter");
  return policy_act(ctx, ob, B, blob, H1, H2, noise_scale, noise, seed, counter_offset, counter, eval_mode, act,
                    mean, x0_buf, stride_m, ldk, row_exp, stride_rexp, slot_stride, n_slots, stream);
}

__global__ void k_counter_add(uint64_t* c, long long d) { c[0] += (uint64_t)d; }

extern "C" int amx_counter_add(amx_ctx* ctx, uint64_t* counter, long long delta, void* stream) {
  AMX_CHECK_ARG(ctx && counter, "amx_counter_add: null pointer");
  hipLaunchKernelGGL(k_counter_add, dim3(1), dim3(1), 0, (hipStream_t)stream, counter, delta);
  AMX_CHECK_LAUNCH();
  return AMX_OK;
}

extern "C" int amx_philox(amx_ctx* ctx, uint64_t seed, uint32_t ctr1, uint32_t ctr2, uint32_t ctr3, uint32_t* out,
                          int n, void* stream) {
  AMX_CHECK_ARG(ctx && out && n >= 0, "amx_philox: bad argument");
  if (n == 0) return AMX_OK;
  hipLaunchKernelGGL(k_philox, dim3((n + 255) / 256), dim3(256), 0, (hipStream_t)stream, (uint32_t)seed,
                     (uint32_t)(seed >> 32), ctr1, ctr2, ctr3, out, n);
  AMX_CHECK_LAUNCH();
  return AMX_OK;
}

extern "C" int amx_set_step_act_occupancy(amx_ctx* ctx, int two_per_cu) {
  AMX_CHECK_ARG(ctx, "amx_set_step_act_occupancy: null ctx");
  ctx->step_act_w8 = two_per_cu ? 1 : 0;
  return AMX_OK;
}
```

### amp_extensions_amd/rollout.py

```python
from __future__ import annotations

import ctypes as C
import math

import numpy as np
import torch

from . import _native as N
from .costs import GAILCost, RBFLinearCost, input_width
from .engine import DeviceEnsemble, round_up
from .humanoid import TerminationConfig
from .policy import DevicePolicy


_CAPTURE_MODE = "thread_local"

class RolloutEngine:
    def __init__(self, ensemble: DeviceEnsemble, reset_table, lanes: int, term: TerminationConfig | None = None,
                 policy: DevicePolicy | None = None, cost=None, seed: int = 0, max_steps: int = 16,
                 eval_mode: bool = False, auto_reset: bool = True, record_means: bool = False):
        self.ens = ensemble
        self.ctx = c = ensemble.ctx
        self.term = term or TerminationConfig()
        c.set_termination(self.term)
        self.B = int(lanes)
        self.Bp = round_up(self.B, 128)
        self.K = int(max_steps)
        self.policy = policy
        self.cost = cost
        self.eval_mode = eval_mode
        self.auto_reset = auto_reset
        self.fuse_reset = True
        self.fuse_assembly = False
        self.fuse_step_act = False
        self._act_ready = -1
        self.seed = int(seed) & 0xFFFFFFFFFFFFFFFF
        dev = c.device
        from .motion import ReferenceMotion
        self.motion = reset_table if isinstance(reset_table, ReferenceMotion) else None
        self.reset_time_max = 0.0
        self.table = None
        if self.motion is None:
            table = torch.as_tensor(reset_table, dtype=torch.float64)
            if table.dim() != 2 or table.shape[1] != c.S:
                raise ValueError(f"reset table must be [R, {c.S}] float64 (or a ReferenceMotion)")
            self.table = table.to(dev).contiguous()
        S, A, B, Bp, K = c.S, c.A, self.B, self.Bp, self.K
        z = lambda *shape, dt=torch.float32: torch.zeros(*shape, dtype=dt, device=dev)
        self.obs = z(K + 1, B, S, dt=torch.float64)
        self.next_obs = z(K, B, S, dt=torch.float64) if auto_reset else self.obs[1:]
        self.acts = z(K, B, A, dt=torch.float64)
        self.done = z(K, B, dt=torch.uint8)
        self.disc = z(K, Bp)
        self.rewards = z(K, Bp)
        self.ipm = z(K, Bp)
        self.wbonus = z(K, Bp)
        self.nonfinite = z(K, B, dt=torch.uint8)
        self.num_steps = z(B, dt=torch.int32)
        self.steps0 = z(B, dt=torch.int32)
        self.model_idx = z(B, dt=torch.int32)
        self.reset_count = z(B, dt=torch.int32)
        self.reset_rows = z(K, B, dt=torch.int32)
        self.reset_times = z(K, B, dt=torch.float64) if self.motion is not None else None
        self.cost_type = getattr(cost, "input_type", "ss") if cost is not None else "ss"
        if isinstance(cost, RBFLinearCost):
            self.kc = cost.map.Kp
        elif isinstance(cost, GAILCost):
            self.kc = cost.Kin
        else:
            self.kc = c.k_rff_pad
        if cost is not None:
            width = input_width(self.cost_type, S, A, getattr(cost, "motion", None))
            if cost.input_dim != width:
                raise ValueError(f"cost input width {cost.input_dim} does not match input_type "
                                 f"{self.cost_type!r} (S={S}, A={A}: {width})")
        self.cost_in = z(K, Bp, self.kc)
        if self.cost_type == "amp" and cost.motion.ctx is not c:
            raise ValueError("the cost's ReferenceMotion must live on the engine's context")
        self.row_mask = None
        if B != Bp:
            self.row_mask = ((torch.arange(K * Bp, device=dev) % Bp) < B).to(torch.uint8)
        self._scored = 0
        self.means = z(K, B, A) if record_means else None
        self.cost_rexp = None
        if (isinstance(cost, RBFLinearCost) and cost.map.W2 is not None) or \
                (isinstance(cost, GAILCost) and cost.gemm == "f16x3"):
            self.cost_rexp = z(K, Bp, dt=torch.int32)
        if isinstance(cost, RBFLinearCost):
            self.phi = z(K, Bp, cost.feature_dim)
            self.partials = z(K, Bp // N.RFF_PART_ROWS, cost.feature_dim, dt=torch.float64)
        self.t = 0
        self.step_counter = 0
        self.dev_step = torch.zeros(1, dtype=torch.int64, device=dev)
        self._capturing = False
        self._ctr_delta = 0
        self._ctr_folded = False
        self._carry = 0
        self._pending = None
        self._graph_ahead = False
        self._fbuf = z(cost.feature_dim + 1, dt=torch.float64) if isinstance(cost, RBFLinearCost) else None
        if self._fbuf is not None:
            self.phi_sum = self._fbuf[:cost.feature_dim]
        self.mb_mmd = None
        self.score_overlap = False
        self._side = None
        self.member_blocks = 0

    def reset_all(self, rows: torch.Tensor | None = None) -> None:
        self.reset_lanes(None, rows)

    def set_reset_noise(self, reset_args: dict | None) -> None:
        noise = N.ResetNoise.from_reset_args(reset_args) if reset_args is not None else None
        if noise is not None and self.motion is None:
            raise NotImplementedError("reset noise needs a ReferenceMotion reset source (AddNoise perturbs the "
                                      "kinematic pose / velocity, which a reset-state table does not hold)")
        self._reset_noise = noise

    def _reset_motion(self, mask, times, src, dst, t_out) -> None:
        c = self.ctx
        noise = getattr(self, "_reset_noise", None)
        N.check(c.lib.amx_reset_lanes_motion_noise(c.h, None if mask is None else mask.data_ptr(),
                                                   None if times is None else times.data_ptr(), self.seed,
                                                   float(self.reset_time_max), self.motion.kernel_flags,
                                                   None if noise is None else C.byref(noise), None, 0,
                                                   src.data_ptr(), dst.data_ptr(),
                                                   self.num_steps.data_ptr(), self.model_idx.data_ptr(),
                                                   self.reset_count.data_ptr(),
                                                   None if t_out is None else t_out.data_ptr(),
                                                   self.B, c.stream), "amx_reset_lanes_motion_noise")

    def reset_lanes(self, mask: torch.Tensor | None, rows: torch.Tensor | None = None,
                    t_out: torch.Tensor | None = None) -> None:
        c = self.ctx
        self.begin_rollout()
        dst = self.obs[0]
        if self.motion is not None:
            self._reset_motion(mask, rows, dst, dst, t_out)
            self.t = 0
            return
        N.check(c.lib.amx_reset_lanes(c.h, None if mask is None else mask.data_ptr(), self.table.data_ptr(),
                                      self.table.shape[0], None if rows is None else rows.data_ptr(), self.seed,
                                      dst.data_ptr(), dst.data_ptr(), self.num_steps.data_ptr(),
                                      self.model_idx.data_ptr(), self.reset_count.data_ptr(), None, self.B,
                                      c.stream), "amx_reset_lanes")
        self.t = 0

    def _rollout_begin(self) -> None:
        fused = self.auto_reset and self.motion is None and self.fuse_reset
        if fused and self.t != 0:
            self._carry, self.t, self._scored = self.t, 0, 0
        else:
            self.begin_rollout()

    def begin_rollout(self) -> None:
        if self.t != 0:
            self.obs[0].copy_(self.obs[self.t])
        self.t = 0
        self._scored = 0

    def sync_step_counter(self, to_device: bool = False) -> None:
        if self._graph_ahead:
            self.step_counter = int(self.dev_step.item())
            self._graph_ahead = False
        if to_device:
            self.dev_step.fill_(self.step_counter)

    def step(self, actions: torch.Tensor | None = None, reset_rows: torch.Tensor | None = None,
             noise: torch.Tensor | None = None, act_next: bool = False) -> int:
        front = self._step_front(actions, noise)
        if front[0] == 0 and self._pending is not None:
            pending, self._pending = self._pending, None
            pending()
        fuse = act_next and actions is None and noise is None and reset_rows is None and self._can_act_next()
        return self._step_back(front, reset_rows, act_next=fuse)

    def _can_act_next(self) -> bool:
        return (self.fuse_step_act and self.policy is not None and self.auto_reset and self.motion is None
                and self.fuse_reset and self.ens.W2 is not None and self.ens.shared_x0
                and self.ctx.S <= 256
                and self.t + 1 < self.K)

    def _step_front(self, actions, noise):
        c, t, B = self.ctx, self.t, self.B
        if t >= self.K:
            raise RuntimeError(f"rollout buffer full ({self.K} steps): call begin_rollout()")
        s = c.stream
        fused = self.auto_reset and self.motion is None and self.fuse_reset
        if t == 0 and not fused:
            self.steps0.copy_(self.num_steps)
        src = self._carry if (t == 0 and self._carry) else t
        self._carry = 0
        ob, ob_next, act = self.obs[src], self.next_obs[t], self.acts[t]
        x0_ready = False
        if self._act_ready == t and actions is None and noise is None:
            x0_ready = True
            self._act_ready = -1
        elif actions is not None:
            self._act_ready = -1
            act.copy_(actions)
        else:
            self._act_ready = -1
            if self.policy is None:
                raise RuntimeError("no policy and no actions given")
            if self._graph_ahead and not self._capturing:
                self.sync_step_counter()
            fuse_x0 = self.fuse_assembly and self.ens.W2 is not None and self.ens.shared_x0
            if not fuse_x0:
                ws = None
            elif self.member_blocks:
                ws = self.ens.workspace_blocked(self.member_blocks)
            else:
                ws = self.ens.workspace(B)
            self.policy.act(ob, B, act, t if self._capturing else self.step_counter, noise=noise,
                            eval_mode=self.eval_mode, mean_out=None if self.means is None else self.means[t],
                            counter_dev=self.dev_step if self._capturing else None,
                            x0=None if ws is None else ws["act"], row_exp=None if ws is None else ws["rexp"],
                            shared_x0=fuse_x0)
            x0_ready = fuse_x0
        if self.member_blocks:
            if self.B != self.ctx.M * self.member_blocks:
                raise ValueError("member-blocked stepping needs M * member_blocks lanes")
            return t, src, self.ens.forward_blocked(ob, act, self.member_blocks, x0_ready=x0_ready)
        preds = self.ens.forward_preds(ob, act, B, x0_ready=x0_ready)
        return t, src, preds

    def _step_back(self, front, reset_rows, act_next: bool = False) -> int:
        c, B, s = self.ctx, self.B, self.ctx.stream
        t, src, preds = front
        fused = self.auto_reset and self.motion is None and self.fuse_reset
        ob, ob_next = self.obs[src], self.next_obs[t]
        sP = 0 if self.member_blocks else preds.shape[1] * c.S
        disc = self.disc[t].data_ptr() if c.M >= 2 and not self.member_blocks else None
        if fused and act_next:
            ss = self.cost_type == "ss"
            pol, ws = self.policy, self.ens.workspace(B)
            rx = ws["rexp"]
            N.check(c.lib.amx_step_reset_act(
                c.h, preds.data_ptr(), c.S, sP, self.model_idx.data_ptr(), ob.data_ptr(),
                ob_next.data_ptr(), self.num_steps.data_ptr(), self.done[t].data_ptr(),
                disc, self.cost_in[t].data_ptr() if ss else None, self.kc,
                self.cost_rexp[t].data_ptr() if ss and self.cost_rexp is not None else None,
                self.nonfinite[t].data_ptr(), self.table.data_ptr(), self.table.shape[0], None, self.seed,
                self.obs[t + 1].data_ptr(), self.reset_count.data_ptr(), self.reset_rows[t].data_ptr(),
                self.steps0.data_ptr() if t == 0 else None, self.obs[0].data_ptr() if src != t else None,
                pol.blob.data_ptr(), pol.H1, pol.H2, pol.noise_scale.data_ptr(), pol.seed,
                (t + 1) if self._capturing else (self.step_counter + 1) & 0xFFFFFFFFFFFFFFFF,
                self.dev_step.data_ptr() if self._capturing else None, int(self.eval_mode), self.acts[t + 1].data_ptr(),
                None if self.means is None else self.means[t + 1].data_ptr(), ws["act"].data_ptr(), 0, c.ldk,
                rx.data_ptr(), rx.stride(0), rx.stride(1), rx.shape[1], B, s), "amx_step_reset_act")
            self._ctr_folded = False
            self._act_ready = t + 1
        elif fused:
            ss = self.cost_type == "ss"
            last = self._capturing and self._ctr_delta and t == self._ctr_delta - 1
            ctr, ctr_delta = (self.dev_step, self._ctr_delta) if last else (None, 0)
            N.check(c.lib.amx_step_reset(c.h, preds.data_ptr(), c.S, sP, self.model_idx.data_ptr(),
                                         ob.data_ptr(), ob_next.data_ptr(), self.num_steps.data_ptr(),
                                         self.done[t].data_ptr(), disc,
                                         self.cost_in[t].data_ptr() if ss else None, self.kc,
                                         self.cost_rexp[t].data_ptr() if ss and self.cost_rexp is not None else None,
                                         self.nonfinite[t].data_ptr(), self.table.data_ptr(), self.table.shape[0],
                                         None if reset_rows is None else reset_rows.data_ptr(), self.seed,
                                         self.obs[t + 1].data_ptr(), self.reset_count.data_ptr(),
                                         self.reset_rows[t].data_ptr(), self.steps0.data_ptr() if t == 0 else None,
                                         ctr.data_ptr() if ctr is not None else None, ctr_delta,
                                         self.obs[0].data_ptr() if src != t else None, B, s),
                    "amx_step_reset")
            self._ctr_folded = ctr is not None
        elif self.cost_type == "ss" and self.cost_rexp is not None:
            N.check(c.lib.amx_step_rexp(c.h, preds.data_ptr(), c.S, sP, self.model_idx.data_ptr(),
                                        ob.data_ptr(), ob_next.data_ptr(), self.num_steps.data_ptr(),
                                        self.done[t].data_ptr(), disc,
                                        self.cost_in[t].data_ptr(), self.kc, self.cost_rexp[t].data_ptr(),
                                        self.nonfinite[t].data_ptr(), B, s), "amx_step_rexp")
        else:
            N.check(c.lib.amx_step(c.h, preds.data_ptr(), c.S, sP, self.model_idx.data_ptr(),
                                   ob.data_ptr(), ob_next.data_ptr(), self.num_steps.data_ptr(),
                                   self.done[t].data_ptr(), disc,
                                   self.cost_in[t].data_ptr() if self.cost_type == "ss" else None, self.kc,
                                   self.nonfinite[t].data_ptr(), B, s), "amx_step")
        if self.cost is not None and self.cost_type != "ss":
            self._record_cost_input(t)
        if fused:
            pass
        elif self.auto_reset and self.motion is not None:
            self._reset_motion(self.done[t], reset_rows, ob_next, self.obs[t + 1], self.reset_times[t])
        elif self.auto_reset:
            N.check(c.lib.amx_reset_lanes(c.h, self.done[t].data_ptr(), self.table.data_ptr(), self.table.shape[0],
                                          None if reset_rows is None else reset_rows.data_ptr(), self.seed,
                                          ob_next.data_ptr(), self.obs[t + 1].data_ptr(), self.num_steps.data_ptr(),
                                          self.model_idx.data_ptr(), self.reset_count.data_ptr(),
                                          self.reset_rows[t].data_ptr(), B, s), "amx_reset_lanes")
        elif ob_next.data_ptr() != self.obs[t + 1].data_ptr():
            self.obs[t + 1].copy_(ob_next)
        self.t += 1
        self.step_counter += 1
        return t

    def _record_cost_input(self, t: int) -> None:
        c, B, S, A = self.ctx, self.B, self.ctx.S, self.ctx.A
        ob, nx, act = self.obs[t], self.next_obs[t], self.acts[t]
        typ = self.cost_type
        if typ == "amp":
            N.check(c.lib.amx_state_amp_rows(c.h, ob.data_ptr(), nx.data_ptr(), S, B, 0,
                                             self.cost_in[t].data_ptr(), self.kc, c.stream), "amx_state_amp_rows")
            return
        if typ == "sa":
            segs = ((ob, S, S), (act, A, A), (None, 0, 0))
        elif typ == "sas":
            segs = ((ob, S, S), (act, A, A), (nx, S, S))
        else:
            segs = ((ob, S, S), (None, 0, 0), (None, 0, 0))
        args = []
        for x, ld, w in segs:
            args += [None if x is None else x.data_ptr(), ld, w]
        N.check(c.lib.amx_cost_rows(c.h, *args, B, self.cost_in[t].data_ptr(), self.kc, c.stream), "amx_cost_rows")

    def rollout(self, K: int | None = None) -> int:
        K = self.K if K is None else K
        self._rollout_begin()
        self._act_ready = -1
        side = self._score_stream() if (self.score_overlap and K > 1 and isinstance(self.cost, RBFLinearCost)
                                        and self.cost.map.step_invariant) else None
        for t in range(K):
            self.step(act_next=t + 1 < K)
            if side is not None and t + 1 < K:
                side.wait_stream(torch.cuda.current_stream(self.ctx.device))
                with torch.cuda.stream(side):
                    self.score()
        if side is not None:
            torch.cuda.current_stream(self.ctx.device).wait_stream(side)
        self.score()
        return K * self.B

    def _score_stream(self):
        if self._side is None:
            self._side = torch.cuda.Stream(self.ctx.device)
        return self._side

    def score(self) -> None:
        c, cost, t0, t1, Bp = self.ctx, self.cost, self._scored, self.t, self.Bp
        if t1 <= t0 or cost is None:
            self._scored = t1
            return
        rows = (t1 - t0) * Bp
        x = self.cost_in[t0:t1].view(rows, self.kc)
        if isinstance(cost, RBFLinearCost):
            mask = None if self.row_mask is None else self.row_mask[t0 * Bp:t1 * Bp]
            rexp = None
            if self.cost_rexp is not None and self.cost_type == "ss":
                rexp = self.cost_rexp[t0:t1].view(rows)
            cost.map.features(x, rows, rows, self.phi[t0:t1].view(rows, -1),
                              self.partials[t0:t1].view(rows // N.RFF_PART_ROWS, -1), row_mask=mask, row_exp=rexp)
        elif isinstance(cost, GAILCost):
            rexp = None
            if self.cost_rexp is not None and self.cost_type == "ss":
                rexp = self.cost_rexp[t0:t1].view(rows)
            cost.rewards_from_input(x, rows, rows, self.disc[t0:t1].view(rows) if c.M >= 2 else None,
                                    out=self.rewards[t0:t1].view(rows), row_exp=rexp)
        self._scored = t1

    def feature_sum(self) -> torch.Tensor:
        self.relabel_pre()
        return self.phi_sum

    def relabel(self, allreduce=None) -> dict:
        cost = self.cost
        self.flush_relabel()
        self.score()
        if isinstance(cost, GAILCost):
            return {}
        if not isinstance(cost, RBFLinearCost):
            raise RuntimeError("relabel needs an RBFLinearCost or GAILCost")
        self.relabel_pre()
        if allreduce is not None:
            allreduce(self._fbuf)
        return self.relabel_post()

    def relabel_pre(self) -> torch.Tensor:
        self.score()
        c, cost = self.ctx, self.cost
        n_parts = self.t * (self.Bp // N.RFF_PART_ROWS)
        N.check(c.lib.amx_feature_message(c.h, self.partials.data_ptr(), n_parts, cost.feature_dim,
                                          float(self.t * self.B), self._fbuf.data_ptr(), c.stream),
                "amx_feature_message")
        return self._fbuf

    def relabel_post(self, T: int | None = None) -> dict:
        cost = self.cost
        n = (self.t if T is None else T) * self.Bp
        self.mb_mmd = cost.relabel_device(self._fbuf, self.phi.data_ptr(), cost.feature_dim, self.disc.data_ptr(),
                                          float(self.ens.threshold), self.rewards.data_ptr(), self.ipm.data_ptr(),
                                          self.wbonus.data_ptr(), n)
        return {"mb_mmd": self.mb_mmd}

    def graph_rollout(self, T: int | None = None, allreduce=None, tail=None, before_relabel=None, after=None):
        T = self.K if T is None else T
        if self.t != T:
            raise RuntimeError("run one eager rollout(T) before capturing")
        mmd = isinstance(self.cost, RBFLinearCost)
        c = self.ctx
        self.sync_step_counter(to_device=True)
        graphs = [torch.cuda.CUDAGraph(), torch.cuda.CUDAGraph()]
        side = torch.cuda.Stream(c.device)
        side.wait_stream(torch.cuda.current_stream(c.device))
        with torch.cuda.stream(side):
            self._capturing = True
            self._ctr_delta, self._ctr_folded = T, False
            try:
                with torch.cuda.graph(graphs[0], stream=side, capture_error_mode=_CAPTURE_MODE):
                    self.rollout(T)
                    if not self._ctr_folded:
                        N.check(c.lib.amx_counter_add(c.h, self.dev_step.data_ptr(), T, c.stream), "amx_counter_add")
                    if mmd:
                        self.relabel_pre()
                        if allreduce is None:
                            self.relabel_post()
                    if tail is not None and (allreduce is None or not mmd):
                        tail()
                if mmd and allreduce is not None:
                    with torch.cuda.graph(graphs[1], stream=side, capture_error_mode=_CAPTURE_MODE):
                        self.relabel_post()
                        if tail is not None:
                            tail()
            finally:
                self._capturing = False
                self._ctr_delta = 0
        torch.cuda.current_stream(c.device).wait_stream(side)
        self._graph_ahead = True
        two = mmd and allreduce is not None

        def replay():
            graphs[0].replay()
            if two:
                if before_relabel is not None:
                    before_relabel()
                allreduce(self._fbuf)
                graphs[1].replay()
            if after is not None:
                after()
            self._graph_ahead = True
            return T * self.B
        return replay

    def rollout_overlapped(self, T: int, allreduce_async, tail=None) -> int:
        if not isinstance(self.cost, RBFLinearCost):
            raise RuntimeError("rollout_overlapped is the MMD path (RBFLinearCost)")
        self.rollout(T)
        self.relabel_pre()
        h = allreduce_async(self._fbuf)

        def pending():
            h.wait()
            self.relabel_post(T)
            if tail is not None:
                tail()
        self._pending = pending
        return T * self.B

    def flush_relabel(self) -> None:
        if self._pending is not None:
            pending, self._pending = self._pending, None
            pending()

    def graph_rollout_overlapped(self, T: int, allreduce_async, tail=None, before_relabel=None, after=None):
        if not isinstance(self.cost, RBFLinearCost):
            raise RuntimeError("graph_rollout_overlapped is the MMD path (RBFLinearCost)")
        if self.t != T or self._pending is not None:
            raise RuntimeError("run one eager rollout(T) + relabel before capturing")
        fused = self.auto_reset and self.motion is None and self.fuse_reset
        if not fused:
            raise RuntimeError("graph_rollout_overlapped needs the fused step + table reset")
        c = self.ctx
        self.sync_step_counter(to_device=True)
        graphs = [torch.cuda.CUDAGraph() for _ in range(3)]
        side = torch.cuda.Stream(c.device)
        side.wait_stream(torch.cuda.current_stream(c.device))
        with torch.cuda.stream(side):
            self._capturing = True
            self._ctr_delta, self._ctr_folded = T, False
            try:
                with torch.cuda.graph(graphs[0], stream=side, capture_error_mode=_CAPTURE_MODE):
                    self._rollout_begin()
                    front = self._step_front(None, None)
                with torch.cuda.graph(graphs[1], stream=side, capture_error_mode=_CAPTURE_MODE):
                    self.relabel_post(T)
                    if tail is not None:
                        tail()
                    self._step_back(front, None)
                    for _ in range(T - 1):
                        self.step()
                    self.score()
                    if not self._ctr_folded:
                        N.check(c.lib.amx_counter_add(c.h, self.dev_step.data_ptr(), T, c.stream), "amx_counter_add")
                    self.relabel_pre()
                with torch.cuda.graph(graphs[2], stream=side, capture_error_mode=_CAPTURE_MODE):
                    self.relabel_post(T)
                    if tail is not None:
                        tail()
            finally:
                self._capturing = False
                self._ctr_delta = 0
        torch.cuda.current_stream(c.device).wait_stream(side)
        self._graph_ahead = True
        state = {"h": None}

        def replay():
            graphs[0].replay()
            if state["h"] is not None:
                state["h"].wait()
            if before_relabel is not None:
                before_relabel()
            graphs[1].replay()
            state["h"] = allreduce_async(self._fbuf)
            if after is not None:
                after()
            self._graph_ahead = True
            return T * self.B

        def flush():
            if state["h"] is not None:
                state["h"].wait()
                state["h"] = None
                if before_relabel is not None:
                    before_relabel()
                graphs[2].replay()
                if after is not None:
                    after()
        return replay, flush

    def advantages(self, baseline, gamma: float = 0.995, gae_lambda=0.97, whiten: bool = False,
                   eps: float = 1e-6) -> dict:
        from .gae import gae_grid, whiten_grid
        self.flush_relabel()
        c, T, B = self.ctx, self.t, self.B
        rows = T * B
        obs = self.obs[:T].reshape(rows, c.S)
        end = self.done[:T].reshape(rows)
        v = baseline.predict_grid(rows, T, B, obs, c.S, end, B, t0=self.steps0)
        ret = torch.empty(T, B, dtype=torch.float64, device=c.device)
        adv = torch.empty_like(ret)
        gae_grid(c, T, B, end, self.rewards, self.Bp, v, gamma, gae_lambda, B, ret, adv)
        out = {"values": v[:rows].view(T, B), "returns": ret, "advantages": adv}
        if whiten:
            out["advantages_whitened"], out["adv_stats"] = whiten_grid(c, T, B, adv, B, eps=eps,
                                                                       out=torch.empty_like(adv))
        return out

    def fit_baseline(self, baseline, returns: torch.Tensor, **kw):
        c, T, B = self.ctx, self.t, self.B
        rows = T * B
        if returns.numel() != rows:
            raise ValueError(f"returns holds {returns.numel()} values, the buffers {rows} rows")
        obs = self.obs[:T].reshape(rows, c.S)
        end = self.done[:T].reshape(rows)
        return baseline.fit_grid(rows, T, B, obs, c.S, end, B, returns, t0=self.steps0, **kw)

    def bonus_mmd(self, allreduce=None) -> float:
        self.flush_relabel()
        T, B = self.t, self.B
        cost = -self.rewards[:T, :B].double()
        if allreduce is None:
            mean_cost = cost.mean()
        else:
            m = torch.stack([cost.sum(), torch.full((), float(T * B), dtype=torch.float64, device=cost.device)])
            allreduce(m)
            mean_cost = m[0] / m[1]
        return float(mean_cost.item()) - float(self.cost.get_expert_cost().item())
```

### include/amx_hip.h

```cpp
#ifndef AMX_HIP_H
#define AMX_HIP_H

#include <stdint.h>

#ifdef __cplusplus
extern "C" {
#endif

#define AMX_ABI_VERSION 2
#define AMX_ROW_TILE 128
#define AMX_K_TILE 32
#define AMX_MAX_MODELS 8
#define AMX_MAX_BODIES 32
#define AMX_MT_STATE_BYTES 2512

enum {
  AMX_OK = 0,
  AMX_E_INVAL = -1,
  AMX_E_HIP = -2,
  AMX_E_NOMEM = -3,
  AMX_E_STATE = -4
};

enum { AMX_SHAPE_SPHERE = 0, AMX_SHAPE_CAPSULE = 1, AMX_SHAPE_BOX = 2 };
enum { AMX_ACT_NONE = 0, AMX_ACT_RELU = 1 };
enum { AMX_IN_F64 = 0, AMX_IN_F32 = 1 };
enum { AMX_DISC_LEAST_SQUARES = 0, AMX_DISC_LOG_LIKELIHOOD = 1 };

typedef struct amx_ctx amx_ctx;


amx_ctx* amx_create(int device, int S, int A, int n_models, int hidden, int n_hidden, int feat_dim);
enum { AMX_CONNECT_DENSE = 0, AMX_CONNECT_PLAIN = 1 };
amx_ctx* amx_create_ex(int device, int S, int A, int n_models, int hidden, int n_hidden, int feat_dim,
                       int connect);
int amx_destroy(amx_ctx* ctx);
const char* amx_last_error(void);
int amx_abi_version(void);

int amx_layout(const amx_ctx* ctx, int* k0_pad, int* ldk, int* n_out_pad, int* k_rff_pad);

int amx_set_normalizers(amx_ctx* ctx, const float* mu_s, const float* sd_s, const float* mu_a,
                        const float* sd_a, const float* mu_d, const float* sd_d);

int amx_set_termination(amx_ctx* ctx, int n_bodies, const int32_t* body_id, const int32_t* shape,
                        const double* p0, const double* p1, int record_all_world,
                        int record_world_root_pos, int pos_dim, int rot_dim, int horizon,
                        int vel_check, int vel_offset, double vel_thresh, int record_vel_as_pos,
                        double sampling_rate);


int amx_assemble_input(amx_ctx* ctx, const void* ob, const void* act, int in_dtype, float* act_buf,
                       long long stride_m, int ldk, int B, void* stream);
int amx_assemble_input_rexp(amx_ctx* ctx, const void* ob, const void* act, int in_dtype, float* act_buf,
                            long long stride_m, int ldk, int B, int* row_exp, long long strideRexp,
                            long long slot_stride, int n_slots, void* stream);

int amx_gemm_bias_act(amx_ctx* ctx, int groups, int rows, int N, int K, const float* A, int lda,
                      long long strideA, const float* W, int ldw, long long strideW,
                      const float* bias, long long strideBias, float* C, int ldc, long long strideC,
                      int col_off, int act, void* stream);

int amx_gemm_bias_act_t64(amx_ctx* ctx, int groups, int rows, int N, int K, const float* A, int lda,
                          long long strideA, const float* W, int ldw, long long strideW,
                          const float* bias, long long strideBias, float* C, int ldc,
                          long long strideC, int col_off, int act, void* stream);

int amx_gemm_out_unnorm(amx_ctx* ctx, int groups, int rows, int n_valid, int K, const float* A,
                        int lda, long long strideA, const float* W, int ldw, long long strideW,
                        const float* bias, long long strideBias, float* preds, int ldp,
                        long long strideP, void* stream);

int amx_split_bf16x3(amx_ctx* ctx, int groups, int rows, int K, const float* W, int ldw,
                     long long strideW, uint16_t* W3, long long strideW3, void* stream);
int amx_gemm_bias_act_x6(amx_ctx* ctx, int groups, int rows, int N, int K, const float* A, int lda,
                         long long strideA, const uint16_t* W3, long long strideW3, const float* bias,
                         long long strideBias, float* C, int ldc, long long strideC, int col_off,
                         int act, void* stream);
int amx_gemm_out_unnorm_x6(amx_ctx* ctx, int groups, int rows, int n_valid, int K, const float* A,
                           int lda, long long strideA, const uint16_t* W3, long long strideW3,
                           const float* bias, long long strideBias, float* preds, int ldp,
                           long long strideP, void* stream);

int amx_rff_features_x6(amx_ctx* ctx, int rows, int n_valid, int F, int K, const float* x, int ldx,
                        const uint16_t* W3, const float* b, float scale, float* phi, int ldphi,
                        double* col_partials, const uint8_t* row_mask, void* stream);

int amx_split_f16x2(amx_ctx* ctx, int groups, int rows, int K, const float* W, int ldw,
                    long long strideW, uint16_t* W2, long long strideW2, int* w_exp,
                    long long strideWexp, void* stream);
int amx_row_exponents(amx_ctx* ctx, int groups, int rows, int K, const float* A, int lda,
                      long long strideA, int* row_exp, long long strideRexp, int n_slots,
                      void* stream);
int amx_gemm_bias_act_h3(amx_ctx* ctx, int groups, int rows, int N, int K, const float* A, int lda,
                         long long strideA, const uint16_t* W2, long long strideW2, const int* w_exp,
                         long long strideWexp, const float* bias, long long strideBias, float* C,
                         int ldc, long long strideC, int col_off, int act, const int* row_exp,
                         long long strideRexp, int rexp_slots, int* row_exp_out, int k_shared,
                         void* stream);
int amx_gemm_out_unnorm_h3(amx_ctx* ctx, int groups, int rows, int n_valid, int K, const float* A,
                           int lda, long long strideA, const uint16_t* W2, long long strideW2,
                           const int* w_exp, long long strideWexp, const float* bias,
                           long long strideBias, float* preds, int ldp, long long strideP,
                           const int* row_exp, long long strideRexp, int rexp_slots, int k_shared,
                           void* stream);

int amx_gemm_bias_act_h3_win(amx_ctx* ctx, int groups, int rows, int N, int K, const float* A, int lda,
                             long long strideA, const uint16_t* W2, long long strideW2, const int* w_exp,
                             long long strideWexp, const float* bias, long long strideBias, float* C,
                             int ldc, long long strideC, int col_off, int act, const int* row_exp,
                             long long strideRexp, int rexp_first, int* row_exp_out, int first_layer,
                             void* stream);
int amx_gemm_out_unnorm_h3_win(amx_ctx* ctx, int groups, int rows, int n_valid, int K, const float* A,
                               int lda, long long strideA, const uint16_t* W2, long long strideW2,
                               const int* w_exp, long long strideWexp, const float* bias,
                               long long strideBias, float* preds, int ldp, long long strideP,
                               const int* row_exp, long long strideRexp, int rexp_first, void* stream);

int amx_rff_features_h3(amx_ctx* ctx, int rows, int n_valid, int F, int K, const float* x, int ldx,
                        const uint16_t* W2, const int* w_exp, const int* row_exp, const float* b, float scale,
                        float* phi, int ldphi, double* col_partials, const uint8_t* row_mask, void* stream);

int amx_mlp_features_h3(amx_ctx* ctx, int rows, int n_valid, int F, int K, const float* x, int ldx,
                        const uint16_t* W2, const int* w_exp, const int* row_exp, const float* b, float scale,
                        float* phi, int ldphi, double* col_partials, const uint8_t* row_mask, void* stream);

#define AMX_NOISE_ROT_SLOTS 48
typedef struct amx_reset_noise {
  int noise_bef_rot;
  double noise_min, noise_max, radian;
  int rot_vel_w_pose, vel_noise;
  double interp;
  int knee_rot;
} amx_reset_noise;
int amx_motion_states_noise(amx_ctx* ctx, const double* times, int B, int flags, const amx_reset_noise* noise,
                            const double* draws, long long ld_draws, uint64_t seed, double* ob, long long ldo,
                            void* stream);
int amx_reset_lanes_motion_noise(amx_ctx* ctx, const uint8_t* mask, const double* times, uint64_t seed,
                                 double time_max, int flags, const amx_reset_noise* noise, const double* draws,
                                 long long ld_draws, const double* ob_src, double* ob_out, int32_t* num_steps,
                                 int32_t* model_idx, int32_t* reset_count, double* t_out, int B, void* stream);
int amx_set_motion(amx_ctx* ctx, const double* blob, long long n);
double amx_motion_duration(const amx_ctx* ctx);
int amx_motion_states(amx_ctx* ctx, const double* times, int B, int flags, double* ob, long long ldo,
                      void* stream);
int amx_reset_lanes_motion(amx_ctx* ctx, const uint8_t* mask, const double* times, uint64_t seed,
                           double time_max, int flags, const double* ob_src, double* ob_out, int32_t* num_steps,
                           int32_t* model_idx, int32_t* reset_count, double* t_out, int B, void* stream);

int amx_amp_obs_size(const amx_ctx* ctx);
int amx_state_amp_obs(amx_ctx* ctx, const double* s_prev, const double* s_cur, long long lds, int B,
                      int local_root, double* out, long long ldo, void* stream);
int amx_motion_amp_obs(amx_ctx* ctx, const double* times, double dt, int B, int local_root, double* out,
                       long long ldo, void* stream);
int amx_state_amp_rows(amx_ctx* ctx, const double* s_prev, const double* s_cur, long long lds, int B,
                       int local_root, float* out, long long ldo, void* stream);

int amx_tw_dim(const amx_ctx* ctx);
int amx_state_tw_rows(amx_ctx* ctx, const double* s, long long lds, int B, int flags, double* out,
                      long long ldo, void* stream);
int amx_motion_tw_rows(amx_ctx* ctx, const double* t0, const double* lift, int T, int n, double update_rate,
                       double* out, long long ldo, void* stream);
#define AMX_E_ARG AMX_E_INVAL
enum { AMX_DTW_COST_SQUARED = 0, AMX_DTW_COST_POINTS = 1 };
long long amx_dtw_work(int T, int n_max);
int amx_dtw_align(amx_ctx* ctx, const double* data0, const double* data1, long long ld, int dim, int cost_kind,
                  int n_max,
                  const int32_t* len_host, const int32_t* len, int T, int buffer_size, double* work,
                  double* cost, double* dtw_cost, int32_t* index, double* backtrack_raw, double* backtrack,
                  void* stream);

long long amx_npg_param_count(int S, int A);
int amx_npg_pass(amx_ctx* ctx, int mode, int N, const void* obs, int obs_dtype, long long ldo,
                 const void* act, int act_dtype, long long lda, const double* adv, const float* theta,
                 const float* vec, int rows_per_block, double* partials, void* stream);
int amx_npg_reduce(amx_ctx* ctx, const double* partials, int blocks, int P, double* out, void* stream);
int amx_npg_pass_gated(amx_ctx* ctx, int mode, int N, const void* obs, int obs_dtype, long long ldo,
                       const void* act, int act_dtype, long long lda, const double* adv, const float* theta,
                       const float* vec, int rows_per_block, double* partials, const double* gate, void* stream);
int amx_npg_reduce_gated(amx_ctx* ctx, const double* partials, int blocks, int P, double* out, const double* gate,
                         void* stream);
int amx_npg_pass_ex(amx_ctx* ctx, int mode, int N, const void* obs, int obs_dtype, long long ldo, const void* act,
                    int act_dtype, long long lda, const double* adv, const float* theta, const float* vec,
                    int rows_per_block, double* partials, const double* gate, float* hcache, void* stream);
int amx_npg_pass_dp(amx_ctx* ctx, int mode, int N, const void* obs, int obs_dtype, long long ldo, const void* act,
                    int act_dtype, long long lda, const double* adv, const float* theta, const float* vec,
                    int rows_per_block, double* partials, const double* gate, float* hcache, long long n_total,
                    void* stream);

int amx_npg_curvature(amx_ctx* ctx, const float* theta, int P, int A, double* curv, void* stream);
int amx_npg_apply_step(amx_ctx* ctx, int P, int A, const double* vpg, const double* npg, const float* theta,
                       int use_alpha, double alpha, double n_step_size, float min_log_std, float* new_theta,
                       double* scal, void* stream);
long long amx_npg_cg_tail_work(int P);
int amx_npg_cg_tail(amx_ctx* ctx, const double* partials, int blocks, int P, int A, const double* curv,
                    double damping, double tol, double* x, const double* r_in, double* r_out, double* p, float* p32,
                    const double* state_in, double* state_out, double* work, void* stream);
int amx_npg_cg_reduce(amx_ctx* ctx, const double* partials, int blocks, int P, int A, const double* curv,
                      double damping, const double* p, const float* p32, const double* state, double* work,
                      void* stream);
int amx_npg_cg_xrp(amx_ctx* ctx, int P, double tol, double* x, const double* r_in, double* r_out, double* p,
                   float* p32, const double* state_in, double* state_out, const double* work, void* stream);
int amx_npg_pass_cg(amx_ctx* ctx, int N, const void* obs, int obs_dtype, long long ldo, const float* theta,
                    int rows_per_block, double* partials, float* hcache, double tol, double* x, const double* r_in,
                    double* r_out, const double* p_in, double* p_out, float* p32_out, const double* state_in,
                    double* state_out, const double* work, void* stream);
int amx_npg_pass_cg_dp(amx_ctx* ctx, int N, const void* obs, int obs_dtype, long long ldo, const float* theta,
                       int rows_per_block, double* partials, float* hcache, double tol, double* x,
                       const double* r_in, double* r_out, const double* p_in, double* p_out, float* p32_out,
                       const double* state_in, double* state_out, const double* work, long long n_total,
                       void* stream);
int amx_npg_pass_idx(amx_ctx* ctx, int N, int M, const int32_t* row_idx, const void* obs, int obs_dtype,
                     long long ldo, const float* theta, const float* vec, int rows_per_block, double* partials,
                     const double* gate, float* hcache, double* prod_count, void* stream);
int amx_npg_pass_cg_idx(amx_ctx* ctx, int N, int M, const int32_t* row_idx, const void* obs, int obs_dtype,
                        long long ldo, const float* theta, int rows_per_block, double* partials, float* hcache,
                        double tol, double* x, const double* r_in, double* r_out, const double* p_in,
                        double* p_out, float* p32_out, const double* state_in, double* state_out,
                        const double* work, double* prod_count, void* stream);
int amx_npg_ll_blocks(amx_ctx* ctx, int N);
int amx_npg_ll(amx_ctx* ctx, int N, const float* obs, long long ldo, const float* act, long long lda,
               const float* theta, double* partials, float* ll, float* mean, void* stream);
int amx_npg_cg_init(amx_ctx* ctx, int P, const double* b, double* x, double* r, double* p, float* p32,
                    double* state, void* stream);
int amx_npg_cg_init_ls(amx_ctx* ctx, int P, int A, const float* theta, double* curv, const double* b, double* x,
                       double* r, double* p, float* p32, double* state, void* stream);
int amx_npg_cg_step(amx_ctx* ctx, int P, int A, const double* h, const double* curv, double damping,
                    double residual_tol, double* x, double* r, double* p, float* p32, double* state,
                    void* stream);


int amx_step(amx_ctx* ctx, const float* preds, int ldp, long long strideP, const int32_t* model_idx,
             const double* ob, double* ob_next, int32_t* num_steps, uint8_t* done, float* disc,
             float* cost_in, int ldc, uint8_t* nonfinite, int B, void* stream);
int amx_step_rexp(amx_ctx* ctx, const float* preds, int ldp, long long strideP, const int32_t* model_idx,
                  const double* ob, double* ob_next, int32_t* num_steps, uint8_t* done, float* disc,
                  float* cost_in, int ldc, int* cost_rexp, uint8_t* nonfinite, int B, void* stream);

int amx_step_reset(amx_ctx* ctx, const float* preds, int ldp, long long strideP, int32_t* model_idx,
                   const double* ob, double* ob_next, int32_t* num_steps, uint8_t* done, float* disc,
                   float* cost_in, int ldc, int* cost_rexp, uint8_t* nonfinite, const double* table,
                   int R, const int32_t* rows, uint64_t seed, double* ob_out, int32_t* reset_count,
                   int32_t* row_out, int32_t* steps0_out, uint64_t* counter, long long counter_delta,
                   double* ob_rec, int B, void* stream);

int amx_step_reset_act(amx_ctx* ctx, const float* preds, int ldp, long long strideP, int32_t* model_idx,
                       const double* ob, double* ob_next, int32_t* num_steps, uint8_t* done, float* disc,
                       float* cost_in, int ldc, int* cost_rexp, uint8_t* nonfinite, const double* table,
                       int R, const int32_t* rows, uint64_t seed, double* ob_out, int32_t* reset_count,
                       int32_t* row_out, int32_t* steps0_out, double* ob_rec, const float* blob, int H1,
                       int H2, const double* noise_scale, uint64_t policy_seed, uint64_t counter,
                       const uint64_t* counter_dev, int eval_mode, double* act, float* mean,
                       float* x0_buf, long long stride_m, int ldk, int* row_exp, long long stride_rexp,
                       long long slot_stride, int n_slots, int B, void* stream);
int amx_set_step_act_occupancy(amx_ctx* ctx, int two_per_cu);

int amx_disagreement(amx_ctx* ctx, const float* preds, int ldp, long long strideP, float* disc,
                     int B, void* stream);

int amx_reset_lanes(amx_ctx* ctx, const uint8_t* mask, const double* table, int R,
                    const int32_t* rows, uint64_t seed, const double* ob_src, double* ob_out,
                    int32_t* num_steps, int32_t* model_idx, int32_t* reset_count, int32_t* row_out,
                    int B, void* stream);


int amx_policy_act(amx_ctx* ctx, const double* ob, int B, const float* blob, int H1, int H2,
                   const double* noise_scale, const double* noise, uint64_t seed, uint64_t counter,
                   int eval_mode, double* act, float* mean, float* x0_buf, long long stride_m, int ldk,
                   int* row_exp, long long stride_rexp, long long slot_stride, int n_slots,
                   void* stream);

int amx_policy_act_dev(amx_ctx* ctx, const double* ob, int B, const float* blob, int H1, int H2,
                       const double* noise_scale, const double* noise, uint64_t seed,
                       const uint64_t* counter, uint64_t counter_offset, int eval_mode, double* act,
                       float* mean, float* x0_buf, long long stride_m, int ldk, int* row_exp,
                       long long stride_rexp, long long slot_stride, int n_slots, void* stream);
int amx_counter_add(amx_ctx* ctx, uint64_t* counter, long long delta, void* stream);

int amx_set_gemm_timer(amx_ctx* ctx, uint64_t* buf);

long long amx_split_workspace_floats(const amx_ctx* ctx, int groups, int rows, int* n_counters);

int amx_set_split_workspace(amx_ctx* ctx, float* scratch, long long floats, uint32_t* counters,
                            int n_counters);

long long amx_policy_blob_floats(const amx_ctx* ctx, int H1, int H2);

int amx_policy_pack(amx_ctx* ctx, const float* W1, const float* b1, int H1, const float* W2,
                    const float* b2, int H2, const float* W3, const float* b3, float* blob,
                    void* stream);


#define AMX_RFF_PART_ROWS 32

int amx_rff_features(amx_ctx* ctx, int rows, int n_valid, int F, int K, const float* x, int ldx,
                     const float* W, int ldw, const float* b, float scale, float* phi, int ldphi,
                     double* col_partials, const uint8_t* row_mask, void* stream);

int amx_sum_partials(amx_ctx* ctx, const double* partials, int n_parts, int F, double* out,
                     void* stream);

int amx_mmd_fit(amx_ctx* ctx, const double* phi_sum, double count, const float* phi_e, int F,
                float* w, float* mmd, void* stream);

int amx_mmd_reward(amx_ctx* ctx, const float* phi, int ldphi, const float* w, int F, const float* disc,
                   float thr, double lambda_b, float c_min, float c_max, float* reward, float* ipm,
                   float* wbonus, int n, void* stream);

int amx_mmd_reward_raw(amx_ctx* ctx, const float* phi, int ldphi, const float* w, int F, const float* disc,
                       double lambda_b, float* reward, float* ipm, float* wbonus, int n, void* stream);

int amx_expert_cost(amx_ctx* ctx, const float* phi_e_rows, int ldphi, const float* w, int F, int n,
                    float c_min, float c_max, double* out, float* mean_out, double lambda_b,
                    void* stream);

int amx_feature_message(amx_ctx* ctx, const double* partials, int n_parts, int F, double count,
                        double* out, void* stream);

int amx_mmd_relabel(amx_ctx* ctx, const double* msg, double count, const float* phi_e, int F,
                    float* w, float* mmd, const float* phi, int ldphi, const float* disc, float thr,
                    double lambda_b, int clamp, float c_min, float c_max, float* reward, float* ipm,
                    float* wbonus, int n, const float* expert_rows, int ld_e, int n_e,
                    double* expert_out, float* expert_mean, uint32_t* counter, void* stream);


int amx_amp_reward(amx_ctx* ctx, const float* h, int ldh, int Hd, const float* w3, float b3,
                   const float* disc, double lambda_b, float* reward, float* logits, int n,
                   void* stream);

int amx_disc_reward(amx_ctx* ctx, int loss_type, const float* h, int ldh, int Hd, const float* w3, float b3,
                    const float* disc, double lambda_b, float* reward, float* logits, int n, void* stream);

int amx_cost_rows(amx_ctx* ctx, const double* x0, long long ld0, int w0, const double* x1, long long ld1, int w1,
                  const double* x2, long long ld2, int w2, int B, float* out, int ldc, void* stream);



int amx_value_features(amx_ctx* ctx, int T, int L, const int32_t* len, const int32_t* t0,
                       const int64_t* base, long long stride, const uint8_t* end,
                       const double* obs, int ldo, float* feat, int ldf, void* stream);

int amx_value_head(amx_ctx* ctx, int rows, const float* h, int ldh, int H, const float* w,
                   const float* b, float* v, void* stream);

int amx_gae(amx_ctx* ctx, int T, int L, const int32_t* len, const int64_t* base, long long stride,
            const uint8_t* end, const float* rew, const int64_t* rbase, long long rstride,
            const float* v, double gamma, double gamma_lambda, double* ret, double* adv,
            void* stream);

int amx_adv_whiten(amx_ctx* ctx, int T, int L, const int32_t* len, const int64_t* base,
                   long long stride, const double* adv, double eps, double* out, double* stats,
                   void* stream);
int amx_adv_whiten_parts(amx_ctx* ctx, int T, int L, const int32_t* len, const int64_t* base, long long stride,
                         const double* adv, int rank, int world, double* msg, void* stream);
int amx_adv_whiten_apply(amx_ctx* ctx, int T, int L, const int32_t* len, const int64_t* base, long long stride,
                         const double* adv, const double* msg, int world, double eps, double* out, double* stats,
                         void* stream);


long long amx_vfit_work(int kf, int H0p, int H1p);
long long amx_vfit_param_count(int kf, int H0p, int H1p);

int amx_vfit_epoch(amx_ctx* ctx, int n_rows, const float* feat, int ldf, const float* returns,
                   const int32_t* perm, int kf, int H0p, int H1p, float* W0, float* b0, float* W1,
                   float* b1, float* w2, float* b2, float* adam_m, float* adam_v,
                   long long* adam_step, double lr, double beta1, double beta2, double eps,
                   double weight_decay, void* work, float* epoch_loss, void* stream);


enum { AMX_EFIT_ADAM = 0, AMX_EFIT_SGD = 1 };

long long amx_efit_param_count(const amx_ctx* ctx);
long long amx_efit_work_floats(const amx_ctx* ctx, int Bt);

int amx_efit_step(amx_ctx* ctx, int train, int n_b, int Bt, const int32_t* idx, long long strideIdx,
                  int n_rows, const float* states, const float* actions, const float* next_states,
                  float* const* W, float* const* b, float* grad, float* state1, float* state2,
                  long long* step, int optim, double lr, double p1, double grad_clip, float* loss,
                  long long strideLoss, float* work, void* stream);


enum { AMX_DFIT_SGD = 0, AMX_DFIT_ADAM = 1 };

int amx_gemm_nn_f32(amx_ctx* ctx, int M, int N, int K, const float* A, int lda, const float* B,
                    int ldb, float* C, int ldc, const float* mask, int ldm, int mask_mod,
                    void* stream);
int amx_gemm_tn_f32(amx_ctx* ctx, int R, int M, int N, const float* A, int lda, const float* B,
                    int ldb, float* C, int ldc, const float* mask, int ldm, float* colsum,
                    int colsum_rows, void* stream);

long long amx_dfit_param_count(int Dp, int H0p, int H1p);
long long amx_dfit_work_floats(int Dp, int H0p, int H1p, int Bt);

int amx_dfit_step(amx_ctx* ctx, int loss_type, int optim, double lr, double p1, double scaling_coef,
                  double reg_coef, double grad_lambda, int bs, int Bt, int D, int Dp, int H0p,
                  int H1p, const int32_t* idx_e, const int32_t* idx_m, const float* expert,
                  long long ld_expert, int n_expert, const float* agent, long long ld_agent,
                  int n_agent, float* W0, float* b0, float* W1, float* b1, float* w2, float* b2,
                  float* state1, float* state2, long long* step, float* work, double* metrics,
                  void* stream);


enum { AMX_BC_MSE = 0, AMX_BC_MLE = 1 };

long long amx_bcfit_work(int S, int A);

int amx_bcfit_steps(amx_ctx* ctx, int N, const float* obs, long long ldo, const float* act,
                    long long lda, const int32_t* idx, int n_steps, float* theta, float* adam_m,
                    float* adam_v, long long* adam_step, double lr, double beta1, double beta2,
                    double eps, double weight_decay, int loss_type, float* step_loss,
                    void* stream);

int amx_bcfit_eval(amx_ctx* ctx, int N, const float* obs, long long ldo, const float* act,
                   long long lda, const float* theta, int loss_type, void* work, double* loss,
                   void* stream);


enum { AMX_PPO_OLD_SNAPSHOT = 0, AMX_PPO_OLD_TRACKS_MEAN = 1 };

int amx_ppo_steps(amx_ctx* ctx, int N, const float* obs, long long ldo, const float* act,
                  long long lda, const float* adv, const float* ll_old, const float* log_std_old,
                  int old_mode, const int32_t* idx, int n_steps, float* theta, float* adam_m,
                  float* adam_v, long long* adam_step, double lr, double beta1, double beta2,
                  double eps, double clip_coef, float* step_loss, int32_t* step_clipped,
                  void* stream);

int amx_ppo_old_ll(amx_ctx* ctx, int N, const float* obs, long long ldo, const float* act,
                   long long lda, const float* theta, float* ll_old, void* stream);


int amx_philox(amx_ctx* ctx, uint64_t seed, uint32_t ctr1, uint32_t ctr2, uint32_t ctr3,
               uint32_t* out, int n, void* stream);

int amx_mt_seed(void* states, int n_states, const int32_t* slots, const uint32_t* seeds, int n);
int amx_mt_policy_noise(void* states, int n_states, const int32_t* slots, int n, int steps, int A,
                        double* out, long long ld_step, long long ld_slot);

#ifdef __cplusplus
}
#endif
#endif
```

Measured before the change: 16.46 million.

## Add step+policy kernel that overlaps record writes with next-action compute

Adds a new fused kernel path, amx_step_rec_act, which splits the step lane logic into load, update, record, done and next-row phases. Waves 4 and up of a 512-thread block write trajectory records while the first four waves run the policy MLP for the next action, with an idle callback that keeps the barriers matched. The rollout enables this path by default when the existing step/act fusion is off. The x0 normalisation loop is also rewritten to handle four columns per thread with an alignment check so stores can be vectorised. The cost is more code paths, tighter eligibility conditions, and register pressure from larger blocks.

Measured after the change: 16.46 million. No clear change (-0.0%).

```diff
diff --git a/amp_extensions_amd/_native.py b/amp_extensions_amd/_native.py
--- a/amp_extensions_amd/_native.py
+++ b/amp_extensions_amd/_native.py
@@ -114,6 +114,9 @@
     "amx_step_reset_act": (c_int, [vp, vp, c_int, c_ll, vp, vp, vp, vp, vp, vp, vp, c_int, vp, vp, vp, c_int, vp,
                                    c_u64, vp, vp, vp, vp, vp, vp, c_int, c_int, vp, c_u64, c_u64, vp, c_int, vp, vp,
                                    vp, c_ll, c_int, vp, c_ll, c_ll, c_int, c_int, vp]),
+    "amx_step_rec_act": (c_int, [vp, vp, c_int, c_ll, vp, vp, vp, vp, vp, vp, vp, c_int, vp, vp, vp, c_int, vp,
+                                 c_u64, vp, vp, vp, vp, vp, vp, c_int, c_int, vp, c_u64, c_u64, vp, c_int, vp, vp,
+                                 vp, c_ll, c_int, vp, c_ll, c_ll, c_int, c_int, vp]),
     "amx_set_step_act_occupancy": (c_int, [vp, c_int]),
     "amx_rff_features_h3": (c_int, [vp, c_int, c_int, c_int, c_int, vp, c_int, vp, vp, vp, vp, c_flt, vp, c_int,
                                     vp, vp, vp]),
diff --git a/amp_extensions_amd/csrc/amx_step.hip b/amp_extensions_amd/csrc/amx_step.hip
--- a/amp_extensions_amd/csrc/amx_step.hip
+++ b/amp_extensions_amd/csrc/amx_step.hip
@@ -151,57 +151,98 @@
   double* ob_rec;
 };
 
+
 template <int NIT, bool MM4>
-__device__ __forceinline__ void step_lane(const StepArgs& a, int b, int lane, float* srow) {
-  const amx_termination& T = a.term;
-  const int S = a.S;
-  const int k = a.model_idx[b];
-  const int ns0 = a.num_steps[b];
-  const int rc0 = a.ob_out ? a.reset_count[b] : 0;
-  const int row0 = (a.ob_out && a.rows) ? a.rows[b] : 0;
-  const double* ob = a.ob + (long long)b * S;
-  double* on = a.ob_next + (long long)b * S;
-
-  double o[NIT], x[NIT];
+struct LaneIn {
+  double o[NIT];
   float p[NIT];
   float pm[MM4 ? 4 : 1][NIT];
+  int k, ns0, rc0, row0;
+};
+
+template <int NIT, bool MM4>
+__device__ __forceinline__ void step_load_counters(const StepArgs& a, int b, LaneIn<NIT, MM4>& in) {
+  in.k = a.model_idx[b];
+  in.ns0 = a.num_steps[b];
+  in.rc0 = a.ob_out ? a.reset_count[b] : 0;
+  in.row0 = (a.ob_out && a.rows) ? a.rows[b] : 0;
+}
+
+template <int NIT, bool MM4>
+__device__ __forceinline__ void step_load_rows(const StepArgs& a, int b, int lane, LaneIn<NIT, MM4>& in) {
+  const int S = a.S;
+  const double* ob = a.ob + (long long)b * S;
   if constexpr (MM4) {
     const float* pb = a.preds + (long long)b * a.ldp;
 #pragma unroll
     for (int it = 0; it < NIT; ++it) {
       const int j = lane + 64 * it;
-      o[it] = j < S ? ob[j] : 0.0;
-#pragma unroll
-      for (int m = 0; m < 4; ++m) pm[m][it] = j < S ? pb[m * a.strideP + j] : 0.f;
-    }
+      in.o[it] = j < S ? ob[j] : 0.0;
+#pragma unroll
+      for (int m = 0; m < 4; ++m) in.pm[m][it] = j < S ? pb[m * a.strideP + j] : 0.f;
+    }
+    const int k = in.k;
 #pragma unroll
     for (int it = 0; it < NIT; ++it)
-      p[it] = k == 0 ? pm[0][it] : k == 1 ? pm[1][it] : k == 2 ? pm[2][it] : pm[3][it];
+      in.p[it] = k == 0 ? in.pm[0][it] : k == 1 ? in.pm[1][it] : k == 2 ? in.pm[2][it] : in.pm[3][it];
   } else {
-    const float* pk = a.preds + (long long)k * a.strideP + (long long)b * a.ldp;
+    const float* pk = a.preds + (long long)in.k * a.strideP + (long long)b * a.ldp;
 #pragma unroll
     for (int it = 0; it < NIT; ++it) {
       const int j = lane + 64 * it;
-      o[it] = j < S ? ob[j] : 0.0;
-      p[it] = j < S ? pk[j] : 0.f;
-    }
-  }
+      in.o[it] = j < S ? ob[j] : 0.0;
+      in.p[it] = j < S ? pk[j] : 0.f;
+    }
+  }
+}
+
+template <int NIT, bool MM4>
+__device__ __forceinline__ void step_load(const StepArgs& a, int b, int lane, LaneIn<NIT, MM4>& in) {
+  step_load_counters<NIT, MM4>(a, b, in);
+  step_load_rows<NIT, MM4>(a, b, lane, in);
+}
+
+struct LaneOut {
+  bool vel_bad, bad;
+  bool dn, nf, reset;
+  int row;
+  float d;
+};
+
+template <int NIT, bool MM4>
+__device__ __forceinline__ void step_update(const StepArgs& a, int lane, const LaneIn<NIT, MM4>& in, double* x,
+                                            LaneOut& r) {
+  const amx_termination& T = a.term;
   const bool vscale = T.vel_check && T.record_vel_as_pos;
-  bool vel_bad = false, bad = false;
-  uint32_t cmax = 0;
+  r.vel_bad = false;
+  r.bad = false;
 #pragma unroll
   for (int it = 0; it < NIT; ++it) {
     const int j = lane + 64 * it;
-    double v = o[it] + (double)p[it];
+    double v = in.o[it] + (double)in.p[it];
     if (vscale && j >= T.vel_offset) v = v / T.sampling_rate;
     x[it] = v;
+    if (j < a.S) {
+      if (T.vel_check && j >= T.vel_offset) r.vel_bad |= fabs(v) > T.vel_thresh;
+      r.bad |= !isfinite(v);
+    }
+  }
+}
+
+template <int NIT>
+__device__ __forceinline__ void step_record_rows(const StepArgs& a, int b, int lane, const double* o,
+                                                 const double* x) {
+  const int S = a.S;
+  double* on = a.ob_next + (long long)b * S;
+  uint32_t cmax = 0;
+#pragma unroll
+  for (int it = 0; it < NIT; ++it) {
+    const int j = lane + 64 * it;
     if (j < S) {
-      on[j] = v;
+      on[j] = x[it];
       if (a.ob_rec) a.ob_rec[(long long)b * S + j] = o[it];
-      if (T.vel_check && j >= T.vel_offset) vel_bad |= fabs(v) > T.vel_thresh;
-      bad |= !isfinite(v);
       if (a.cost_in) {
-        const float c0 = (float)o[it], c1 = (float)v;
+        const float c0 = (float)o[it], c1 = (float)x[it];
         a.cost_in[(long long)b * a.ldc + j] = c0;
         a.cost_in[(long long)b * a.ldc + S + j] = c1;
         const uint32_t u0 = __float_as_uint(c0) & 0x7fffffffu, u1 = __float_as_uint(c1) & 0x7fffffffu;
@@ -224,16 +265,20 @@
       }
     }
   }
-
+}
+
+template <int NIT>
+__device__ __forceinline__ void step_done(const StepArgs& a, int lane, const double* x, int ns0, LaneOut& r) {
+  const amx_termination& T = a.term;
   auto fetch = [&](int j) -> double {
     const int src = j & 63, itj = j >> 6;
-    double r = 0.0;
+    double v0 = 0.0;
 #pragma unroll
     for (int it = 0; it < NIT; ++it) {
       const double v = __shfl(x[it], src);
-      r = (itj == it) ? v : r;
-    }
-    return r;
+      v0 = (itj == it) ? v : v0;
+    }
+    return v0;
   };
   const int bi = lane < T.n ? lane : 0;
   const double root_y = fetch(0);
@@ -253,22 +298,28 @@
     }
   }
   const bool collided = __ballot(hit) != 0ull;
-  const bool vexp = __ballot(vel_bad) != 0ull;
-  const bool nf = __ballot(bad) != 0ull;
-
+  const bool vexp = __ballot(r.vel_bad) != 0ull;
+  r.nf = __ballot(r.bad) != 0ull;
+  const bool horizon_done = ns0 + 1 >= T.horizon;
+  r.dn = horizon_done || collided || vexp;
+}
+
+template <int NIT, bool MM4>
+__device__ __forceinline__ float step_disagreement(const StepArgs& a, int b, int lane,
+                                                   const LaneIn<NIT, MM4>& in) {
   float d = 0.f;
   if constexpr (MM4) {
     if (a.disc) {
       double acc[6] = {0.0, 0.0, 0.0, 0.0, 0.0, 0.0};
 #pragma unroll
       for (int it = 0; it < NIT; ++it) {
-        if (lane + 64 * it < S) {
+        if (lane + 64 * it < a.S) {
           int q = 0;
 #pragma unroll
           for (int i = 0; i < 4; ++i)
 #pragma unroll
             for (int kk = i + 1; kk < 4; ++kk) {
-              const float df = pm[i][it] - pm[kk][it];
+              const float df = in.pm[i][it] - in.pm[kk][it];
               acc[q++] += (double)df * (double)df;
             }
         }
@@ -282,57 +333,97 @@
       d = (float)sqrt(mx);
     }
   } else {
-    if (a.disc) d = disagreement_dispatch(a.M, a.preds, a.strideP, a.ldp, b, S, lane);
-  }
-
+    if (a.disc) d = disagreement_dispatch(a.M, a.preds, a.strideP, a.ldp, b, a.S, lane);
+  }
+  return d;
+}
+
+template <int NIT>
+__device__ __forceinline__ void step_next_row(const StepArgs& a, int b, int lane, const double* x, int rc0, int row0,
+                                              double* oo, float* srow, LaneOut& r) {
+  const int S = a.S;
+  r.reset = false;
+  r.row = -1;
+  if (!r.dn) {
+#pragma unroll
+    for (int it = 0; it < NIT; ++it) {
+      const int j = lane + 64 * it;
+      if (j < S) {
+        if (oo) oo[j] = x[it];
+        if (srow) srow[j] = (float)x[it];
+      }
+    }
+  } else {
+    r.reset = true;
+    const int rc = rc0 + 1;
+    int row;
+    if (a.rows) {
+      row = row0;
+    } else {
+      const amx::u32x4 rr = amx::philox4x32_10({(uint32_t)b, (uint32_t)rc, 0u, amx::kTagReset}, a.k0, a.k1);
+      row = (int)((((uint64_t)rr.y << 32) | rr.x) % (uint64_t)a.R);
+    }
+    r.row = row;
+    const double* src = a.table + (long long)row * S;
+    for (int j = lane; j < S; j += 64) {
+      const double v = src[j];
+      if (oo) oo[j] = v;
+      if (srow) srow[j] = (float)v;
+    }
+  }
+}
+
+__device__ __forceinline__ void step_record_flags(const StepArgs& a, int b, int lane, int ns0, int rc0,
+                                                  const LaneOut& r) {
+  if (a.counter && b == 0 && lane == 0) a.counter[0] += (uint64_t)a.counter_delta;
+  if (lane != 0) return;
+  if (a.ob_out) {
+    if (r.reset) {
+      const int rc = rc0 + 1;
+      a.reset_count[b] = rc;
+      a.model_idx_out[b] = rc % a.M;
+    }
+    if (a.row_out) a.row_out[b] = r.row;
+  }
   const int ns = ns0 + 1;
-  const bool horizon_done = ns >= T.horizon;
-  const bool dn = horizon_done || collided || vexp;
-  bool reset = false;
-  if (a.ob_out) {
-    double* oo = a.ob_out + (long long)b * S;
-    if (!dn) {
-#pragma unroll
-      for (int it = 0; it < NIT; ++it) {
-        const int j = lane + 64 * it;
-        if (j < S) {
-          oo[j] = x[it];
-          if (srow) srow[j] = (float)x[it];
-        }
-      }
-      if (lane == 0 && a.row_out) a.row_out[b] = -1;
-    } else {
-      reset = true;
-      const int rc = rc0 + 1;
-      int row;
-      if (a.rows) {
-        row = row0;
-      } else {
-        const amx::u32x4 r = amx::philox4x32_10({(uint32_t)b, (uint32_t)rc, 0u, amx::kTagReset}, a.k0, a.k1);
-        row = (int)((((uint64_t)r.y << 32) | r.x) % (uint64_t)a.R);
-      }
-      const double* src = a.table + (long long)row * S;
-      for (int j = lane; j < S; j += 64) {
-        const double v = src[j];
-        oo[j] = v;
-        if (srow) srow[j] = (float)v;
-      }
-      if (lane == 0) {
-        a.reset_count[b] = rc;
-        a.model_idx_out[b] = rc % a.M;
-        if (a.row_out) a.row_out[b] = row;
-      }
-    }
-  }
-
-  if (a.counter && b == 0 && lane == 0) a.counter[0] += (uint64_t)a.counter_delta;
-  if (lane == 0) {
-    if (a.steps0_out) a.steps0_out[b] = ns - 1;
-    a.num_steps[b] = reset ? 0 : ns;
-    a.done[b] = dn ? 1 : 0;
-    if (a.disc) a.disc[b] = d;
-    if (a.nonfinite) a.nonfinite[b] = nf ? 1 : 0;
-  }
+  if (a.steps0_out) a.steps0_out[b] = ns - 1;
+  a.num_steps[b] = r.reset ? 0 : ns;
+  a.done[b] = r.dn ? 1 : 0;
+  if (a.disc) a.disc[b] = r.d;
+  if (a.nonfinite) a.nonfinite[b] = r.nf ? 1 : 0;
+}
+
+template <int NIT, bool MM4>
+__device__ __forceinline__ LaneOut step_records(const StepArgs& a, int b, int lane, const LaneIn<NIT, MM4>& in,
+                                                float* srow) {
+  LaneOut r;
+  double x[NIT];
+  step_update<NIT, MM4>(a, lane, in, x, r);
+  step_record_rows<NIT>(a, b, lane, in.o, x);
+  step_done<NIT>(a, lane, x, in.ns0, r);
+  r.d = step_disagreement<NIT, MM4>(a, b, lane, in);
+  r.reset = false;
+  r.row = -1;
+  if (a.ob_out) step_next_row<NIT>(a, b, lane, x, in.rc0, in.row0, a.ob_out + (long long)b * a.S, srow, r);
+  return r;
+}
+
+template <int NIT, bool MM4>
+__device__ __forceinline__ void step_lane(const StepArgs& a, int b, int lane, float* srow) {
+  LaneIn<NIT, MM4> in;
+  step_load<NIT, MM4>(a, b, lane, in);
+  const LaneOut r = step_records<NIT, MM4>(a, b, lane, in, srow);
+  step_record_flags(a, b, lane, in.ns0, in.rc0, r);
+}
+
+template <int NIT>
+__device__ __forceinline__ void step_next_obs(const StepArgs& a, int b, int lane, const LaneIn<NIT, false>& in,
+                                              float* srow) {
+  LaneOut r;
+  double x[NIT];
+  step_update<NIT, false>(a, lane, in, x, r);
+  step_done<NIT>(a, lane, x, in.ns0, r);
+  step_next_row<NIT>(a, b, lane, x, in.rc0, in.row0, nullptr, srow, r);
 }
 
 template <int NIT, bool MM4>
@@ -506,7 +597,23 @@
   }
 }
 
-__device__ __forceinline__ void policy_core(const PolicyArgs& p, float* psm, int b0, int img_floats) {
+constexpr int POL_STAGES = 7;
+struct PolNoIdle {
+  __device__ void operator()(int) const {}
+};
+
+template <class Idle>
+__device__ __forceinline__ void pol_follow(bool x0, Idle&& idle) {
+#pragma unroll
+  for (int i = 0; i < POL_STAGES; ++i) {
+    if (i == POL_STAGES - 1 && !x0) break;
+    idle(i);
+    __syncthreads();
+  }
+}
+
+template <class Idle>
+__device__ __forceinline__ void policy_core(const PolicyArgs& p, float* psm, int b0, int img_floats, Idle&& idle) {
   const int S = p.S, A = p.A, H1 = p.H1, H2 = p.H2;
   const int s1 = pol_stride(S), s2 = pol_stride(H1), s3 = pol_stride(H2);
   float* w1 = psm;
@@ -522,7 +629,10 @@
   float* xa_s = mo + POL_LANES * A;
   float* part = xa_s + POL_LANES * A;
   const int t = threadIdx.x;
-  const bool on = t < 256;
+  if (__builtin_amdgcn_readfirstlane(t >> 6) >= 4) {
+    pol_follow(p.x0 != nullptr, idle);
+    return;
+  }
   const int nc1 = (S + 3) >> 2, nc2 = (H1 + 3) >> 2, nc3 = (H2 + 3) >> 2;
   const int npairs = (A + 1) >> 1;
   constexpr int POL_PRE = 2;
@@ -534,22 +644,22 @@
 #pragma unroll
     for (int h = 0; h < 2; ++h) {
       const int u = 2 * pr + h;
-      const bool ok = on && e < POL_LANES * npairs && b < p.B && u < A;
+      const bool ok = e < POL_LANES * npairs && b < p.B && u < A;
       pre_n[q][h] = (ok && p.noise && !p.eval_mode) ? p.noise[(long long)b * A + u] : 0.0;
       pre_s[q][h] = (ok && !p.eval_mode) ? p.nscale[u] : 0.0;
     }
   }
-  if (on) pol_mfma_layer(so, s1, nc1, w1, s1, H1, part);
+  pol_mfma_layer(so, s1, nc1, w1, s1, H1, part);
   __syncthreads();
-  if (on) pol_combine(part, H1, nc1, bb1, true, h1, s2);
+  pol_combine(part, H1, nc1, bb1, true, h1, s2);
   __syncthreads();
-  if (on) pol_mfma_layer(h1, s2, nc2, w2, s2, H2, part);
+  pol_mfma_layer(h1, s2, nc2, w2, s2, H2, part);
   __syncthreads();
-  if (on) pol_combine(part, H2, nc2, bb2, true, h2, s3);
+  pol_combine(part, H2, nc2, bb2, true, h2, s3);
   __syncthreads();
-  if (on) pol_mfma_layer(h2, s3, nc3, w3, s3, A, part);
+  pol_mfma_layer(h2, s3, nc3, w3, s3, A, part);
   __syncthreads();
-  if (on) pol_combine(part, A, nc3, bb3, false, mo, A);
+  pol_combine(part, A, nc3, bb3, false, mo, A);
   __syncthreads();
   uint32_t ctr_lo = p.ctr_lo, ctr_hi = p.ctr_hi;
   if (p.ctr_dev) {
@@ -589,15 +699,12 @@
       if (p.x0) xa_s[l * A + u] = (float)a_out;
     }
   };
-  if (on) {
-#pragma unroll
-    for (int q = 0; q < POL_PRE; ++q)
-      if (t + 256 * q < POL_LANES * npairs) act_item(t + 256 * q, pre_n[q], pre_s[q]);
-    for (int e = t + 256 * POL_PRE; e < POL_LANES * npairs; e += 256) act_item(e, nullptr, nullptr);
-  }
+#pragma unroll
+  for (int q = 0; q < POL_PRE; ++q)
+    if (t + 256 * q < POL_LANES * npairs) act_item(t + 256 * q, pre_n[q], pre_s[q]);
+  for (int e = t + 256 * POL_PRE; e < POL_LANES * npairs; e += 256) act_item(e, nullptr, nullptr);
   if (!p.x0) return;
   __syncthreads();
-  if (!on) return;
   const float* mu_s = p.norm;
   const float* sd_s = p.norm + S;
   const float* mu_a = p.norm + 2 * S;
@@ -607,36 +714,53 @@
   const int ll = t >> 4, c0 = t & 15;
   const int bb = b0 + ll;
   const bool row_ok = bb < p.B;
-  constexpr int QT = POL_X0_COLS / 16;
-  float mu[QT], sd[QT];
-#pragma unroll
-  for (int q = 0; q < QT; ++q) {
-    const int j = c0 + 16 * q;
-    mu[q] = 0.f;
-    sd[q] = 1.f;
-    if (j < S) {
-      mu[q] = mu_s[j];
-      sd[q] = sd_s[j];
-    } else if (j < S + A) {
-      mu[q] = mu_a[j - S];
-      sd[q] = sd_a[j - S];
-    }
-  }
+  const bool vec = ((reinterpret_cast<uintptr_t>(p.x0) & 15) | (p.ldk & 3) | (p.stride_m & 3) | (k0 & 3)) == 0;
+  constexpr int QT = POL_X0_COLS / 64;
+  float mu[QT][4], sd[QT][4];
+#pragma unroll
+  for (int q = 0; q < QT; ++q)
+#pragma unroll
+    for (int e = 0; e < 4; ++e) {
+      const int j = 4 * (c0 + 16 * q) + e;
+      mu[q][e] = 0.f;
+      sd[q][e] = 1.f;
+      if (j < S) {
+        mu[q][e] = mu_s[j];
+        sd[q][e] = sd_s[j];
+      } else if (j < S + A) {
+        mu[q][e] = mu_a[j - S];
+        sd[q][e] = sd_a[j - S];
+      }
+    }
   uint32_t mx = 0;
   if (row_ok) {
 #pragma unroll
     for (int q = 0; q < QT; ++q) {
-      const int j = c0 + 16 * q;
-      if (j >= k0) break;
-      float x = 0.f;
-      if (j < S) {
-        x = (so[ll * s1 + j] - mu[q]) / sd[q];
-      } else if (j < S + A) {
-        x = (xa_s[ll * A + j - S] - mu[q]) / sd[q];
-      }
-      for (int mm = 0; mm < copies; ++mm) p.x0[mm * p.stride_m + (long long)bb * p.ldk + j] = x;
-      const uint32_t bits = __float_as_uint(x) & 0x7fffffffu;
-      mx = mx > bits ? mx : bits;
+      const int j0 = 4 * (c0 + 16 * q);
+      if (j0 >= k0) break;
+      float x[4];
+#pragma unroll
+      for (int e = 0; e < 4; ++e) {
+        const int j = j0 + e;
+        x[e] = 0.f;
+        if (j < S) {
+          x[e] = (so[ll * s1 + j] - mu[q][e]) / sd[q][e];
+        } else if (j < S + A) {
+          x[e] = (xa_s[ll * A + j - S] - mu[q][e]) / sd[q][e];
+        }
+        const uint32_t bits = __float_as_uint(x[e]) & 0x7fffffffu;
+        if (j < k0) mx = mx > bits ? mx : bits;
+      }
+      for (int mm = 0; mm < copies; ++mm) {
+        float* dst = p.x0 + mm * p.stride_m + (long long)bb * p.ldk + j0;
+        if (vec) {
+          *reinterpret_cast<pf4*>(dst) = pf4{x[0], x[1], x[2], x[3]};
+        } else {
+#pragma unroll
+          for (int e = 0; e < 4; ++e)
+            if (j0 + e < k0) dst[e] = x[e];
+        }
+      }
     }
   }
   if (p.row_exp == nullptr) return;
@@ -674,7 +798,7 @@
   pol_stage_all(psm, p.blob, nblob >> 2, so, s1, p.ob + (long long)b0 * S, nl * S, S);
   for (int i = t; i < POL_LANES * (s2 + s3); i += 256) h1[i] = 0.f;
   __syncthreads();
-  policy_core(p, psm, b0, nblob);
+  policy_core(p, psm, b0, nblob, PolNoIdle{});
 }
 
 __host__ __device__ inline int pol_image_lds_floats(int S, int H1, int H2, int A) {
@@ -703,7 +827,69 @@
   }
   for (int i = t; i < POL_LANES * (s2 + s3); i += 1024) h1[i] = 0.f;
   __syncthreads();
-  policy_core(p, psm, b0, nimg);
+  policy_core(p, psm, b0, nimg, PolNoIdle{});
+}
+
+constexpr int REC_LANES = POL_LANES / 4;
+
+template <int NIT, bool MM4>
+__global__ __launch_bounds__(512) __attribute__((amdgpu_waves_per_eu(4))) void k_step_rec_act(StepArgs a,
+                                                                                              PolicyArgs p) {
+  extern __shared__ __attribute__((aligned(16))) float psm[];
+  const int S = p.S, s1 = pol_stride(S), s2 = pol_stride(p.H1), s3 = pol_stride(p.H2);
+  const int nimg = pol_image_lds_floats(S, p.H1, p.H2, p.A);
+  float* so = psm + nimg;
+  float* h1 = so + POL_LANES * s1;
+  const int t = threadIdx.x, lane = t & 63, wave = __builtin_amdgcn_readfirstlane(t >> 6);
+  const int b0 = blockIdx.x * POL_LANES;
+  for (int q = wave; q < (nimg >> 8); q += 8)
+    __builtin_amdgcn_global_load_lds((const __attribute__((address_space(1))) void*)(p.blob + q * 256 + 4 * lane),
+                                     (__attribute__((address_space(3))) void*)(psm + q * 256), 16, 0, 0);
+  for (int i = t; i < POL_LANES * (s2 + s3); i += 512) h1[i] = 0.f;
+  const int lb = b0 + REC_LANES * (wave & 3);
+  LaneIn<NIT, MM4> cur, nxt;
+  LaneOut first;
+  auto record = [&](int i, bool flags) __attribute__((always_inline)) {
+    if (i + 1 < REC_LANES && lb + i + 1 < a.B) step_load<NIT, MM4>(a, lb + i + 1, lane, nxt);
+    if (lb + i < a.B) {
+      const LaneOut r = step_records<NIT, MM4>(a, lb + i, lane, cur, nullptr);
+      if (flags) step_record_flags(a, lb + i, lane, cur.ns0, cur.rc0, r);
+      else first = r;
+    }
+  };
+  if (wave < 4) {
+    LaneIn<NIT, false> in[REC_LANES];
+#pragma unroll
+    for (int i = 0; i < REC_LANES; ++i)
+      if (lb + i < a.B) step_load_counters<NIT, false>(a, lb + i, in[i]);
+#pragma unroll
+    for (int i = 0; i < REC_LANES; ++i)
+      if (lb + i < a.B) step_load_rows<NIT, false>(a, lb + i, lane, in[i]);
+#pragma unroll
+    for (int i = 0; i < REC_LANES; ++i) {
+      float* srow = so + (REC_LANES * wave + i) * s1;
+      if (lb + i < a.B) {
+        step_next_obs<NIT>(a, lb + i, lane, in[i], srow);
+        for (int j = S + lane; j < s1; j += 64) srow[j] = 0.f;
+      } else {
+        for (int j = lane; j < s1; j += 64) srow[j] = 0.f;
+      }
+    }
+  } else {
+    if (lb < a.B) step_load<NIT, MM4>(a, lb, lane, cur);
+    record(0, false);
+  }
+  __syncthreads();
+  policy_core(p, psm, b0, nimg, [&](int stage) __attribute__((always_inline)) {
+    if (stage == 0) {
+      if (lb < a.B) step_record_flags(a, lb, lane, cur.ns0, cur.rc0, first);
+      cur = nxt;
+      record(1, true);
+    } else if (stage + 1 < REC_LANES) {
+      cur = nxt;
+      record(stage + 1, true);
+    }
+  });
 }
 
 __global__ void k_policy_pack(const float* __restrict__ W1, const float* __restrict__ b1, int H1,
@@ -859,7 +1045,7 @@
 static int step_impl(amx_ctx* ctx, const float* preds, int ldp, long long strideP, const int32_t* model_idx,
                      const double* ob, double* ob_next, int32_t* num_steps, uint8_t* done, float* disc,
                      float* cost_in, int ldc, int* cost_rexp, uint8_t* nonfinite, int B, void* stream,
-                     const ResetArgs* rs = nullptr, const PolicyArgs* pa = nullptr) {
+                     const ResetArgs* rs = nullptr, const PolicyArgs* pa = nullptr, bool rec_act = false) {
   AMX_CHECK_ARG(ctx && ctx->have_term, "amx_step: context has no termination config");
   AMX_CHECK_ARG(preds && model_idx && ob && ob_next && num_steps && done, "amx_step: null pointer");
   AMX_CHECK_ARG(ldp >= ctx->S && B >= 0, "amx_step: ldp=%d B=%d", ldp, B);
@@ -897,6 +1083,21 @@
                                 pol_blob_floats(ctx->S, pa->H1, pa->H2, ctx->A)) * sizeof(float);
     AMX_CHECK_ARG(lds <= 160 * 1024, "amx_step_reset_act: S/H too large for LDS staging (%zu B)", lds);
     const dim3 grid((B + POL_LANES - 1) / POL_LANES);
+    if (rec_act) {
+      AMX_CHECK_ARG(pa->x0 && rs->ob_out != ob, "amx_step_rec_act: needs x0_buf, and ob_out must differ from ob");
+      switch (nit) {
+#define AMX_STEP_REC_CASE(N)                                                                                       \
+  case N:                                                                                                          \
+    if (ctx->M == 4) hipLaunchKernelGGL((k_step_rec_act<N, true>), grid, dim3(512), lds, (hipStream_t)stream, a,    \
+                                        *pa);                                                                      \
+    else hipLaunchKernelGGL((k_step_rec_act<N, false>), grid, dim3(512), lds, (hipStream_t)stream, a, *pa);        \
+    break;
+        AMX_STEP_REC_CASE(1) AMX_STEP_REC_CASE(2) AMX_STEP_REC_CASE(3) AMX_STEP_REC_CASE(4)
+#undef AMX_STEP_REC_CASE
+      }
+      AMX_CHECK_LAUNCH();
+      return AMX_OK;
+    }
     switch (nit) {
 #define AMX_STEP_ACT_CASE(N)                                                                                       \
   case N:                                                                                                          \
@@ -976,6 +1177,27 @@
                    nonfinite, B, stream, &rs, &p);
 }
 
+extern "C" int amx_step_rec_act(amx_ctx* ctx, const float* preds, int ldp, long long strideP, int32_t* model_idx,
+                                const double* ob, double* ob_next, int32_t* num_steps, uint8_t* done, float* disc,
+                                float* cost_in, int ldc, int* cost_rexp, uint8_t* nonfinite, const double* table,
+                                int R, const int32_t* rows, uint64_t seed, double* ob_out, int32_t* reset_count,
+                                int32_t* row_out, int32_t* steps0_out, double* ob_rec, const float* blob, int H1,
+                                int H2, const double* noise_scale, uint64_t policy_seed, uint64_t counter,
+                                const uint64_t* counter_dev, int eval_mode, double* act, float* mean,
+                                float* x0_buf, long long stride_m, int ldk, int* row_exp, long long stride_rexp,
+                                long long slot_stride, int n_slots, int B, void* stream) {
+  AMX_CHECK_ARG(!cost_rexp || cost_in, "amx_step_rec_act: cost_rexp needs cost_in");
+  PolicyArgs p;
+  int rc = make_policy_args("amx_step_rec_act", ctx, nullptr, B, blob, H1, H2, noise_scale, nullptr, policy_seed,
+                            counter, counter_dev, eval_mode, act, mean, x0_buf, stride_m, ldk, row_exp, stride_rexp,
+                            slot_stride, n_slots, p);
+  if (rc) return rc;
+  const ResetArgs rs = {table, R, rows, seed, ob_out, model_idx, reset_count, row_out, steps0_out, nullptr, 0,
+                        ob_rec};
+  return step_impl(ctx, preds, ldp, strideP, model_idx, ob, ob_next, num_steps, done, disc, cost_in, ldc, cost_rexp,
+                   nonfinite, B, stream, &rs, &p, true);
+}
+
 extern "C" int amx_disagreement(amx_ctx* ctx, const float* preds, int ldp, long long strideP, float* disc, int B,
                                 void* stream) {
   AMX_CHECK_ARG(ctx && preds && disc, "amx_disagreement: null pointer");
diff --git a/amp_extensions_amd/rollout.py b/amp_extensions_amd/rollout.py
--- a/amp_extensions_amd/rollout.py
+++ b/amp_extensions_amd/rollout.py
@@ -33,6 +33,7 @@
         self.fuse_reset = True
         self.fuse_assembly = False
         self.fuse_step_act = False
+        self.overlap_records = True
         self._act_ready = -1
         self.seed = int(seed) & 0xFFFFFFFFFFFFFFFF
         dev = c.device
@@ -167,18 +168,30 @@
 
     def step(self, actions: torch.Tensor | None = None, reset_rows: torch.Tensor | None = None,
              noise: torch.Tensor | None = None, act_next: bool = False) -> int:
+        if act_next and self.member_blocks:
+            raise ValueError("member-blocked stepping cannot compute the next action in the step kernel "
+                             "(act_next / rollout()): use step()")
         front = self._step_front(actions, noise)
         if front[0] == 0 and self._pending is not None:
             pending, self._pending = self._pending, None
             pending()
-        fuse = act_next and actions is None and noise is None and reset_rows is None and self._can_act_next()
-        return self._step_back(front, reset_rows, act_next=fuse)
+        free = act_next and actions is None and noise is None and reset_rows is None
+        fuse = free and self._can_act_next()
+        rec = free and not fuse and self._can_rec_act(front[1])
+        return self._step_back(front, reset_rows, act_next=fuse, rec_act=rec)
 
     def _can_act_next(self) -> bool:
         return (self.fuse_step_act and self.policy is not None and self.auto_reset and self.motion is None
                 and self.fuse_reset and self.ens.W2 is not None and self.ens.shared_x0
                 and self.ctx.S <= 256
                 and self.t + 1 < self.K)
+
+    def _can_rec_act(self, src: int) -> bool:
+        return (self.overlap_records and not self._capturing and not self.member_blocks
+                and self.policy is not None and self.auto_reset and self.motion is None
+                and self.fuse_reset and self.ens.W2 is not None and self.ens.shared_x0
+                and self.cost_type == "ss" and self.ctx.S <= 256
+                and self.t + 1 < self.K and src != self.t + 1)
 
     def _step_front(self, actions, noise):
         c, t, B = self.ctx, self.t, self.B
@@ -224,18 +237,19 @@
         preds = self.ens.forward_preds(ob, act, B, x0_ready=x0_ready)
         return t, src, preds
 
-    def _step_back(self, front, reset_rows, act_next: bool = False) -> int:
+    def _step_back(self, front, reset_rows, act_next: bool = False, rec_act: bool = False) -> int:
         c, B, s = self.ctx, self.B, self.ctx.stream
         t, src, preds = front
         fused = self.auto_reset and self.motion is None and self.fuse_reset
         ob, ob_next = self.obs[src], self.next_obs[t]
         sP = 0 if self.member_blocks else preds.shape[1] * c.S
         disc = self.disc[t].data_ptr() if c.M >= 2 and not self.member_blocks else None
-        if fused and act_next:
+        if fused and (act_next or rec_act):
             ss = self.cost_type == "ss"
             pol, ws = self.policy, self.ens.workspace(B)
             rx = ws["rexp"]
-            N.check(c.lib.amx_step_reset_act(
+            name = "amx_step_rec_act" if rec_act else "amx_step_reset_act"
+            N.check(getattr(c.lib, name)(
                 c.h, preds.data_ptr(), c.S, sP, self.model_idx.data_ptr(), ob.data_ptr(),
                 ob_next.data_ptr(), self.num_steps.data_ptr(), self.done[t].data_ptr(),
                 disc, self.cost_in[t].data_ptr() if ss else None, self.kc,
@@ -247,7 +261,7 @@
                 (t + 1) if self._capturing else (self.step_counter + 1) & 0xFFFFFFFFFFFFFFFF,
                 self.dev_step.data_ptr() if self._capturing else None, int(self.eval_mode), self.acts[t + 1].data_ptr(),
                 None if self.means is None else self.means[t + 1].data_ptr(), ws["act"].data_ptr(), 0, c.ldk,
-                rx.data_ptr(), rx.stride(0), rx.stride(1), rx.shape[1], B, s), "amx_step_reset_act")
+                rx.data_ptr(), rx.stride(0), rx.stride(1), rx.shape[1], B, s), name)
             self._ctr_folded = False
             self._act_ready = t + 1
         elif fused:
diff --git a/include/amx_hip.h b/include/amx_hip.h
--- a/include/amx_hip.h
+++ b/include/amx_hip.h
@@ -253,6 +253,15 @@
                        const uint64_t* counter_dev, int eval_mode, double* act, float* mean,
                        float* x0_buf, long long stride_m, int ldk, int* row_exp, long long stride_rexp,
                        long long slot_stride, int n_slots, int B, void* stream);
+int amx_step_rec_act(amx_ctx* ctx, const float* preds, int ldp, long long strideP, int32_t* model_idx,
+                     const double* ob, double* ob_next, int32_t* num_steps, uint8_t* done, float* disc,
+                     float* cost_in, int ldc, int* cost_rexp, uint8_t* nonfinite, const double* table,
+                     int R, const int32_t* rows, uint64_t seed, double* ob_out, int32_t* reset_count,
+                     int32_t* row_out, int32_t* steps0_out, double* ob_rec, const float* blob, int H1,
+                     int H2, const double* noise_scale, uint64_t policy_seed, uint64_t counter,
+                     const uint64_t* counter_dev, int eval_mode, double* act, float* mean,
+                     float* x0_buf, long long stride_m, int ldk, int* row_exp, long long stride_rexp,
+                     long long slot_stride, int n_slots, int B, void* stream);
 int amx_set_step_act_occupancy(amx_ctx* ctx, int two_per_cu);
 
 int amx_disagreement(amx_ctx* ctx, const float* preds, int ldp, long long strideP, float* disc,
```
